# Hypersonic-cpu/DSP-AudioRecLabs

Measured on NVIDIA B200. Metric: audio-seconds processed/sec (features+endpoints+KNN), higher is better.
Workload: dtype i16->f32/f64

## Files before the change

### dsp_audioreclabs_b200/csrc/capi.cu

```cuda
#include <cmath>
#include <cstdarg>
#include <cstdio>
#include <cstdlib>
#include <cstring>
#include <string>
#include <vector>

#include "kernels.cuh"
#include "knn.cuh"
#include "mfcc_dtw.cuh"
#include "misc.cuh"

using namespace dsp;

namespace {

thread_local std::string g_err;

int fail(int code, const char* fmt, ...) {
  char buf[512];
  va_list ap;
  va_start(ap, fmt);
  vsnprintf(buf, sizeof buf, fmt, ap);
  va_end(ap);
  g_err = buf;
  return code;
}

#define CU(expr)                                                                         \
  do {                                                                                   \
    cudaError_t e__ = (expr);                                                            \
    if (e__ != cudaSuccess)                                                              \
      return fail(DSP_ERR_CUDA, "%s failed: %s (%s:%d)", #expr, cudaGetErrorString(e__), \
                  __FILE__, __LINE__);                                                   \
  } while (0)

struct DevBuf {
  void* p = nullptr;
  size_t cap = 0;
  cudaError_t ensure(size_t bytes) {
    if (bytes <= cap) return cudaSuccess;
    if (p) cudaFree(p);
    p = nullptr; cap = 0;
    size_t want = bytes + bytes / 8 + 256;
    cudaError_t e = cudaMalloc(&p, want);
    if (e == cudaSuccess) cap = want;
    return e;
  }
  void release() { if (p) cudaFree(p); p = nullptr; cap = 0; }
  template <class T> T* as() const { return reinterpret_cast<T*>(p); }
};

struct PinBuf {
  void* p = nullptr;
  size_t cap = 0;
  cudaError_t ensure(size_t bytes) {
    if (bytes <= cap) return cudaSuccess;
    if (p) cudaFreeHost(p);
    p = nullptr; cap = 0;
    cudaError_t e = cudaMallocHost(&p, bytes + 256);
    if (e == cudaSuccess) cap = bytes + 256;
    return e;
  }
  void release() { if (p) cudaFreeHost(p); p = nullptr; cap = 0; }
  template <class T> T* as() const { return reinterpret_cast<T*>(p); }
};

constexpr size_t kMaxSmemPerCta = 227 * 1024;
constexpr int64_t kFastMaxLen = 1 << 20;
constexpr int kKnnDenseMaxDim = 16384;
constexpr int64_t kKnnDenseQueryChunk = 32768;
constexpr size_t kHostChunkBytesDefault = 512u << 20;
static size_t host_chunk_bytes() {
  static const size_t v = [] { const char* e = std::getenv("DSP_HOST_CHUNK_MB"); const long mb = e ? std::atol(e) : 0; return mb >= 1 && mb <= 4096 ? (size_t)mb << 20 : kHostChunkBytesDefault; }();
  return v;
}

size_t dtype_size(int dtype) {
  switch (dtype) {
    case DSP_S16: return 2;
    case DSP_U8: return 1;
    case DSP_F32: return 4;
    case DSP_F64: return 8;
    default: return 0;
  }
}

struct Slot {
  DevBuf samples, off, foff, eoff, ints, stats, feat, epd_e, epd_z, f64;
  PinBuf h_off;
  cudaEvent_t ev_in = nullptr, ev_k = nullptr, ev_out = nullptr;
  bool busy = false;
};

}

struct dsp_context {
  int device = 0;
  int sm_count = 0;
  cudaStream_t own = nullptr, stream = nullptr, s_in = nullptr, s_out = nullptr;
  int64_t launches = 0;
  struct WinEntry { int type, len; DevBuf w64, w32; };
  std::vector<WinEntry*> windows;
  const double* win64 = nullptr;
  const float* win32 = nullptr;
  DevBuf counters;
  DevBuf flag_list, zbuf, seqbuf;
  size_t occ_smem = 0;
  int occ_variant = -1;
  int pcm_variant = -1;
  int stagger_ns = 0;
  int tma_chunk = 4096;
  int knn_prune = 1;
  int occ = 0;
  Slot slot[2];
  DevBuf tmp[16];
};

struct dsp_knn {
  dsp_context* ctx = nullptr;
  int64_t n = 0, index_base = 0;
  int d = 0, dp = 0, k = 0;
  float tnorm_max = 0.f;
  bool dense = false;
  bool tc16 = false;
  DevBuf tc_train, tc_train_rows, tc_q, tc_flags;
  DevBuf train64, train32, labels, tnorm, cand_idx, cand_worst, qnorm, redo_list, redo_count, nbr_label, q, o_idx, o_dist, o_lab;
  DevBuf refine_list, refine_thr, surv_count, surv_rows;
  DevBuf thr0;
  DevBuf prune_perm, prune_geom, prune_box, prune_ws, prune_bound;
  int64_t prune_tiles = 0;
  DevBuf tpacked, tnorm_dense, qpacked, qnorm_chunk, dense_flags, part_d, part_i;
};

namespace {

int host_window(int type, int n, std::vector<double>& w) {
  if (n < 0) return fail(DSP_ERR_INVALID, "window length must be >= 0");
  w.assign((size_t)n, 1.0);
  if (type == DSP_WIN_RECTANGULAR) return DSP_OK;
  if (type != DSP_WIN_HAMMING && type != DSP_WIN_HANNING)
    return fail(DSP_ERR_INVALID, "unsupported window type: %d", type);
  if (n <= 1) return DSP_OK;
  const double a = type == DSP_WIN_HAMMING ? 0.54 : 0.5, b = type == DSP_WIN_HAMMING ? 0.46 : 0.5;
  for (int i = 0; i < n; ++i) {
    const double m = (double)(1 - n + 2 * i);
    w[(size_t)i] = a + b * std::cos(M_PI * m / (double)(n - 1));
  }
  return DSP_OK;
}

int ensure_window(dsp_context* c, int type, int fl) {
  for (auto* e : c->windows)
    if (e->type == type && e->len == fl) { c->win64 = e->w64.as<double>(); c->win32 = e->w32.as<float>(); return DSP_OK; }
  std::vector<double> w;
  int rc = host_window(type, fl, w);
  if (rc) return rc;
  std::vector<float> wf(w.begin(), w.end());
  if (c->windows.size() >= 256) {
    CU(cudaDeviceSynchronize());
    for (auto* e : c->windows) { e->w64.release(); e->w32.release(); delete e; }
    c->windows.clear();
  }
  auto* e = new dsp_context::WinEntry{type, fl, {}, {}};
  if (e->w64.ensure(sizeof(double) * (size_t)fl + 16) != cudaSuccess || e->w32.ensure(sizeof(float) * (size_t)fl + 16) != cudaSuccess) {
    e->w64.release(); e->w32.release(); delete e;
    return fail(DSP_ERR_NOMEM, "device allocation failed");
  }
  CU(cudaMemcpy(e->w64.p, w.data(), sizeof(double) * (size_t)fl, cudaMemcpyHostToDevice));
  CU(cudaMemcpy(e->w32.p, wf.data(), sizeof(float) * (size_t)fl, cudaMemcpyHostToDevice));
  c->windows.push_back(e);
  c->win64 = e->w64.as<double>(); c->win32 = e->w32.as<float>();
  return DSP_OK;
}

int check_params(const dsp_frontend_params* p) {
  if (!p) return fail(DSP_ERR_INVALID, "params is NULL");
  if (p->frame_length < 1 || p->frame_shift < 1) return fail(DSP_ERR_INVALID, "frame_length and frame_shift must be >= 1");
  if (p->window < 0 || p->window > 2) return fail(DSP_ERR_INVALID, "unsupported window type: %d", p->window);
  if (p->channels != 1 && p->channels != 2) return fail(DSP_ERR_INVALID, "channels must be 1 or 2 (load_wav only down-mixes two channels, audio_processing.py:43-44: pass other files as 1 channel)");
  return DSP_OK;
}

struct ExactExtras {
  int pre_mode = 3, do_features = 1;
  double* pre_out = nullptr;
  double* frames_out = nullptr;
  double* epd_zcr_f64 = nullptr;
  double* feat_f64[3] = {nullptr, nullptr, nullptr};
  double* stats_f64 = nullptr;
};

int launch_exact(dsp_context* c, const void* samples, int dtype, const int64_t* offsets, const int32_t* lengths,
                 const int64_t* feat_offsets, const int64_t* epd_offsets, const int32_t* list,
                 const int32_t* list_count, int64_t n_items, int64_t max_len, const dsp_frontend_params* p,
                 const dsp_frontend_outputs* out, const ExactExtras& ex, int grid) {
  if (grid < 1) grid = 1;
  const int64_t cap_frames = std::max<int64_t>(frame_count_host_device(max_len, p->frame_length, p->frame_shift), 1);
  CU(c->zbuf.ensure(sizeof(double) * (size_t)grid * (size_t)std::max<int64_t>(max_len, 1)));
  CU(c->seqbuf.ensure(sizeof(double) * (size_t)grid * 5 * (size_t)cap_frames));
  ExactArgs a{};
  a.samples = samples; a.dtype = dtype; a.channels = p->channels;
  a.offsets = offsets; a.lengths = lengths; a.feat_offsets = feat_offsets; a.epd_offsets = epd_offsets;
  a.list = list; a.list_count = list_count; a.n_items = n_items;
  a.fl = p->frame_length; a.fs = p->frame_shift;
  a.do_epd = p->do_endpoint_detection; a.pre_mode = ex.pre_mode; a.do_features = ex.do_features;
  a.hr = p->energy_high_ratio; a.lr = p->energy_low_ratio; a.zr = p->zcr_threshold_ratio;
  a.win = c->win64;
  a.zbuf = c->zbuf.as<double>(); a.zbuf_stride = std::max<int64_t>(max_len, 1);
  a.seqbuf = c->seqbuf.as<double>(); a.seq_cap = cap_frames;
  if (out) a.out = *out;
  a.pre_out = ex.pre_out; a.frames_out = ex.frames_out; a.epd_zcr_f64 = ex.epd_zcr_f64;
  a.feat_f64[0] = ex.feat_f64[0]; a.feat_f64[1] = ex.feat_f64[1]; a.feat_f64[2] = ex.feat_f64[2];
  a.stats_f64 = ex.stats_f64;
  frontend_exact_kernel<<<grid, kExactThreads, 0, c->stream>>>(a);
  c->launches++;
  CU(cudaGetLastError());
  return DSP_OK;
}

int frontend_device(dsp_context* c, const void* samples, int dtype, const int64_t* offsets, const int32_t* lengths,
                    const int64_t* feat_offsets, const int64_t* epd_offsets, int64_t B, int64_t max_len,
                    const dsp_frontend_params* p, const dsp_frontend_outputs* out) {
  int rc = check_params(p);
  if (rc) return rc;
  if (!dtype_size(dtype)) return fail(DSP_ERR_INVALID, "unsupported sample dtype %d", dtype);
  if (!out) return fail(DSP_ERR_INVALID, "outputs is NULL");
  if (B < 0 || max_len < 0) return fail(DSP_ERR_INVALID, "negative batch size or length");
  if (B == 0) return DSP_OK;
  if (B > INT32_MAX / 2) return fail(DSP_ERR_UNSUPPORTED, "more than 2^30 utterances in one call");
  if (p->channels == 2 && (dtype == DSP_F32 || dtype == DSP_F64))
    return fail(DSP_ERR_INVALID, "stereo input is only defined for PCM (load_wav)");
  if ((out->energy || out->magnitude || out->zcr) && !feat_offsets) return fail(DSP_ERR_INVALID, "feat_offsets is NULL");
  if ((out->epd_energy || out->epd_zcr) && !epd_offsets) return fail(DSP_ERR_INVALID, "epd_offsets is NULL");
  rc = ensure_window(c, p->window, p->frame_length);
  if (rc) return rc;
  const int fl = p->frame_length, fs = p->frame_shift;
  const int64_t cap_frames64 = std::max<int64_t>(frame_count_host_device(max_len, fl, fs), 1);

  const bool want64 = out->energy_f64 || out->magnitude_f64 || out->zcr_f64 || out->stats_f64 || out->epd_zcr_f64 || out->frames_f64;
  if (out->frames_f64 && !feat_offsets) return fail(DSP_ERR_INVALID, "feat_offsets is NULL");
  if ((out->energy_f64 || out->magnitude_f64 || out->zcr_f64) && !(out->energy_f64 && out->magnitude_f64 && out->zcr_f64))
    return fail(DSP_ERR_INVALID, "energy_f64, magnitude_f64 and zcr_f64 are written together: pass all three or none");
  if (out->energy_f64 && !feat_offsets) return fail(DSP_ERR_INVALID, "feat_offsets is NULL");
  if (out->epd_zcr_f64 && !epd_offsets) return fail(DSP_ERR_INVALID, "epd_offsets is NULL");
  bool fast = dtype == DSP_S16 && p->channels == 1 && !p->force_exact && !want64 && max_len <= kFastMaxLen &&
              feat_offsets;
  size_t smem = 0;
  int cap_samples = 0;
  constexpr int kAutoStream = 2, kAutoResident = 0;
  int variant = (c->pcm_variant >= 0 && c->pcm_variant < pcm_num_variants()) ? c->pcm_variant : (p->aligned16 ? kAutoStream : kAutoResident);
  if (pcm_variant_streams(variant) && !p->aligned16 && c->pcm_variant < 0) variant = kAutoResident;
  const int kPipeVariant = pcm_num_variants();
  PipePlan plan{};
  bool pipe = fast && (c->pcm_variant == kPipeVariant || c->pcm_variant < 0) &&
              pipe_kernel_plan(max_len, (int)cap_frames64, fl, kMaxSmemPerCta, &plan);
  if (fast && !pipe && c->pcm_variant == kPipeVariant) variant = kAutoResident;
  if (pipe) {
    CU(c->counters.ensure(64));
    CU(c->flag_list.ensure(sizeof(int32_t) * (size_t)B));
    CU(cudaMemsetAsync(c->counters.p, 0, 64, c->stream));
    PcmArgs a{};
    a.samples = reinterpret_cast<const int16_t*>(samples);
    a.offsets = offsets; a.lengths = lengths; a.feat_offsets = feat_offsets; a.epd_offsets = epd_offsets;
    a.n_utts = B; a.fl = fl; a.fs = fs; a.window = p->window; a.do_epd = p->do_endpoint_detection;
    a.hr = p->energy_high_ratio; a.lr = p->energy_low_ratio; a.zr = p->zcr_threshold_ratio;
    a.win_f32 = c->win32;
    a.cap_frames = (int)cap_frames64;
    a.tma_chunk = std::getenv("DSP_PIPE_DEBUG") ? std::atoi(std::getenv("DSP_PIPE_DEBUG")) : 0;
    a.ring_slots = plan.ring_slots; a.n_rec = plan.n_rec; a.cap_groups = plan.cap_groups;
    a.sm_count = c->sm_count;
    a.work_counter = c->counters.as<unsigned int>();
    a.flag_count = c->counters.as<int32_t>() + 1;
    a.flag_list = c->flag_list.as<int32_t>();
    a.out = *out;
    const int grid = (int)std::min<int64_t>(B, (int64_t)c->sm_count);
    static long long* d_prof = nullptr;
    if (std::getenv("DSP_PROF")) {
      if (!d_prof) cudaMalloc(&d_prof, 16 * sizeof(long long));
      cudaMemsetAsync(d_prof, 0, 16 * sizeof(long long), c->stream);
      a.prof = d_prof;
    }
    CU(launch_frontend_pipe(a, grid, plan.smem, c->stream));
    if (a.prof) {
      long long h[16]; cudaMemcpyAsync(h, d_prof, sizeof h, cudaMemcpyDeviceToHost, c->stream); cudaStreamSynchronize(c->stream);
      const char* nm[12] = {"S.wait_full", "S.passA", "S.bar1", "S.passB", "S.bar2", "S.wait_rec", "S.passF", "-", "T.wait", "T.decide", "T.window", "T.stats+out"};
      fprintf(stderr, "[prof pipe R=%d nrec=%d] utterances=%lld (cycles/utt, stream warp 0 / tail warp 0 x nrec)", plan.ring_slots, plan.n_rec, h[15]);
      for (int i = 0; i < 12; ++i) fprintf(stderr, "  %s=%.0f", nm[i], (double)h[i] / (double)std::max<long long>(h[15], 1) * (i >= 8 ? plan.n_rec : 1));
      fprintf(stderr, "\n");
    }
    c->launches++;
    ExactExtras ex;
    const int xgrid = (int)std::min<int64_t>(B, (int64_t)c->sm_count);
    return launch_exact(c, samples, dtype, offsets, lengths, feat_offsets, epd_offsets, a.flag_list, a.flag_count, 0,
                        max_len, p, out, ex, xgrid);
  }
  if (fast) {
    cap_samples = (int)((std::max<int64_t>(max_len, 1) + 63) / 64 * 64);
    smem = pcm_kernel_smem_bytes(cap_samples, (int)cap_frames64, fl, !pcm_variant_streams(variant));
    if (smem > kMaxSmemPerCta && !pcm_variant_streams(variant)) fast = false;
    if (smem > kMaxSmemPerCta) fast = false;
  }
  if (!fast) {
    const int grid = (int)std::min<int64_t>(B, (int64_t)c->sm_count * 4);
    ExactExtras ex;
    ex.feat_f64[0] = out->energy_f64; ex.feat_f64[1] = out->magnitude_f64; ex.feat_f64[2] = out->zcr_f64;
    ex.stats_f64 = out->stats_f64; ex.epd_zcr_f64 = out->epd_zcr_f64; ex.frames_out = out->frames_f64;
    return launch_exact(c, samples, dtype, offsets, lengths, feat_offsets, epd_offsets, nullptr, nullptr, B, max_len,
                        p, out, ex, grid);
  }
  if (c->occ_smem != smem || c->occ_variant != variant) {
    c->occ = pcm_kernel_max_ctas_per_sm(variant, smem);
    c->occ_smem = smem;
    c->occ_variant = variant;
    if (c->occ < 1) return fail(DSP_ERR_CUDA, "fast kernel does not fit: %zu bytes of shared memory", smem);
  }
  CU(c->counters.ensure(64));
  CU(c->flag_list.ensure(sizeof(int32_t) * (size_t)B));
  CU(cudaMemsetAsync(c->counters.p, 0, 64, c->stream));
  PcmArgs a{};
  a.samples = reinterpret_cast<const int16_t*>(samples);
  a.offsets = offsets; a.lengths = lengths; a.feat_offsets = feat_offsets; a.epd_offsets = epd_offsets;
  a.n_utts = B; a.fl = fl; a.fs = fs; a.window = p->window; a.do_epd = p->do_endpoint_detection;
  a.hr = p->energy_high_ratio; a.lr = p->energy_low_ratio; a.zr = p->zcr_threshold_ratio;
  a.win_f32 = c->win32;
  a.cap_samples = cap_samples; a.cap_frames = (int)cap_frames64;
  a.tma_chunk = c->tma_chunk;
  a.stagger_ns = c->stagger_ns;
  a.sm_count = c->sm_count;
  a.prof = nullptr;
  static long long* d_prof = nullptr;
  if (std::getenv("DSP_PROF")) {
    if (!d_prof) cudaMalloc(&d_prof, 16 * sizeof(long long));
    cudaMemsetAsync(d_prof, 0, 16 * sizeof(long long), c->stream);
    a.prof = d_prof;
  }
  a.work_counter = c->counters.as<unsigned int>();
  a.flag_count = c->counters.as<int32_t>() + 1;
  a.flag_list = c->flag_list.as<int32_t>();
  a.out = *out;
  const int grid = (int)std::min<int64_t>(B, (int64_t)c->sm_count * c->occ);
  CU(launch_frontend_pcm(variant, a, grid, smem, c->stream));
  if (a.prof) { long long h[16]; cudaMemcpyAsync(h, d_prof, sizeof h, cudaMemcpyDeviceToHost, c->stream); cudaStreamSynchronize(c->stream);
    const char* nm[12] = {"load_wait", "P1", "feat_empty_wait", "P2", "P2b", "P3tail(searches)", "P4", "fixup+handoff", "P3a(select passes)", "P3b(gather)", "P3c(rank+thresholds)", "P3d(N3N4)"};
    double tot = 0; for (int i = 0; i < 12; ++i) tot += (double)h[i];
    fprintf(stderr, "[prof] utterances=%lld", h[15]); for (int i = 0; i < 12; ++i) fprintf(stderr, "  %s=%.0f", nm[i], (double)h[i] / (double)h[15]); fprintf(stderr, "  total=%.0f cycles/utt\n", tot / (double)h[15]); }
  c->launches++;
  ExactExtras ex;
  const int xgrid = (int)std::min<int64_t>(B, (int64_t)c->sm_count);
  return launch_exact(c, samples, dtype, offsets, lengths, feat_offsets, epd_offsets, a.flag_list, a.flag_count, 0,
                      max_len, p, out, ex, xgrid);
}

struct OneShot {
  dsp_context* c;
  int n_tmp = 0;
  explicit OneShot(dsp_context* ctx) : c(ctx) {}
  template <class T> T* dev(size_t count) {
    DevBuf& b = c->tmp[n_tmp++];
    if (b.ensure(sizeof(T) * std::max<size_t>(count, 1)) != cudaSuccess) return nullptr;
    return b.as<T>();
  }
};

}

extern "C" {

int dsp_abi_version(void) { return DSPFRONT_ABI_VERSION; }
const char* dsp_last_error(void) { return g_err.c_str(); }

int dsp_create(int device, dsp_context** out) {
  if (!out) return fail(DSP_ERR_INVALID, "out is NULL");
  *out = nullptr;
  int count = 0;
  if (cudaGetDeviceCount(&count) != cudaSuccess || count == 0) {
    cudaGetLastError();
    return fail(DSP_ERR_NO_DEVICE, "no CUDA device: libdspfront has no CPU path");
  }
  if (device < 0 || device >= count) return fail(DSP_ERR_INVALID, "device %d out of range (%d visible)", device, count);
  CU(cudaSetDevice(device));
  cudaDeviceProp prop;
  CU(cudaGetDeviceProperties(&prop, device));
  if (prop.major < 10) return fail(DSP_ERR_NO_DEVICE, "device %d is sm_%d%d; this library is built for sm_100a only", device, prop.major, prop.minor);
  dsp_context* c = new dsp_context();
  c->device = device;
  c->sm_count = prop.multiProcessorCount;
  CU(cudaStreamCreateWithFlags(&c->own, cudaStreamNonBlocking));
  CU(cudaStreamCreateWithFlags(&c->s_in, cudaStreamNonBlocking));
  CU(cudaStreamCreateWithFlags(&c->s_out, cudaStreamNonBlocking));
  c->stream = c->own;
  if (const char* e = std::getenv("DSP_PCM_VARIANT")) { int v = std::atoi(e); if (v >= -1 && v <= pcm_num_variants()) c->pcm_variant = v; }
  if (const char* e = std::getenv("DSP_STAGGER_NS")) c->stagger_ns = std::atoi(e);
  if (const char* e = std::getenv("DSP_TMA_CHUNK")) { int v = std::atoi(e); if (v >= 16 && v % 16 == 0) c->tma_chunk = v; }
  for (auto& s : c->slot) {
    CU(cudaEventCreateWithFlags(&s.ev_in, cudaEventDisableTiming));
    CU(cudaEventCreateWithFlags(&s.ev_k, cudaEventDisableTiming));
    CU(cudaEventCreateWithFlags(&s.ev_out, cudaEventDisableTiming));
  }
  *out = c;
  return DSP_OK;
}

int dsp_destroy(dsp_context* c) {
  if (!c) return DSP_OK;
  cudaSetDevice(c->device);
  cudaDeviceSynchronize();
  for (auto& s : c->slot) {
    s.samples.release(); s.off.release(); s.foff.release(); s.eoff.release(); s.ints.release();
    s.stats.release(); s.feat.release(); s.epd_e.release(); s.epd_z.release(); s.f64.release(); s.h_off.release();
    if (s.ev_in) cudaEventDestroy(s.ev_in);
    if (s.ev_k) cudaEventDestroy(s.ev_k);
    if (s.ev_out) cudaEventDestroy(s.ev_out);
  }
  for (auto& b : c->tmp) b.release();
  for (auto* e : c->windows) { e->w64.release(); e->w32.release(); delete e; }
  c->windows.clear();
  c->counters.release(); c->flag_list.release();
  c->zbuf.release(); c->seqbuf.release();
  if (c->own) cudaStreamDestroy(c->own);
  if (c->s_in) cudaStreamDestroy(c->s_in);
  if (c->s_out) cudaStreamDestroy(c->s_out);
  delete c;
  return DSP_OK;
}

int dsp_set_stream(dsp_context* c, void* cuda_stream) {
  if (!c) return fail(DSP_ERR_INVALID, "context is NULL");
  c->stream = reinterpret_cast<cudaStream_t>(cuda_stream);
  return DSP_OK;
}

int dsp_use_own_stream(dsp_context* c) {
  if (!c) return fail(DSP_ERR_INVALID, "context is NULL");
  c->stream = c->own;
  return DSP_OK;
}

int dsp_set_tuning(dsp_context* c, const char* key, int value) {
  if (!c || !key) return fail(DSP_ERR_INVALID, "bad argument");
  if (!std::strcmp(key, "pcm_variant")) {
    if (value < -1 || value > pcm_num_variants()) return fail(DSP_ERR_INVALID, "pcm_variant out of range (%d builds + the pipelined kernel)", pcm_num_variants());
    c->pcm_variant = value;
  } else if (!std::strcmp(key, "tma_chunk")) {
    if (value < 16 || value % 16) return fail(DSP_ERR_INVALID, "tma_chunk must be a positive multiple of 16");
    c->tma_chunk = value;
  } else if (!std::strcmp(key, "stagger_ns")) {
    c->stagger_ns = value;
  } else if (!std::strcmp(key, "knn_prune")) {
    if (value < 0 || value > 2) return fail(DSP_ERR_INVALID, "knn_prune must be 0 (off), 1 (automatic) or 2 (always)");
    c->knn_prune = value;
  } else {
    return fail(DSP_ERR_INVALID, "unknown tuning key '%s'", key);
  }
  return DSP_OK;
}

int dsp_sync(dsp_context* c) {
  if (!c) return fail(DSP_ERR_INVALID, "context is NULL");
  CU(cudaSetDevice(c->device));
  CU(cudaStreamSynchronize(c->stream));
  return DSP_OK;
}

int64_t dsp_launch_count(dsp_context* c) { return c ? c->launches : 0; }
int dsp_device_sm_count(dsp_context* c) { return c ? c->sm_count : 0; }

int64_t dsp_frame_count(int64_t n, int32_t fl, int32_t fs) {
  if (fl < 1 || fs < 1) return 0;
  return frame_count_host_device(n, fl, fs);
}

int dsp_frontend_plan(const int64_t* offsets, const int32_t* lengths, int64_t B, const dsp_frontend_params* p,
                      int64_t* feat_offsets, int64_t* epd_offsets, int64_t* max_len) {
  int rc = check_params(p);
  if (rc) return rc;
  if (!offsets || B < 0) return fail(DSP_ERR_INVALID, "bad offsets");
  int64_t fo = 0, eo = 0, mx = 0;
  for (int64_t b = 0; b < B; ++b) {
    const int64_t room = offsets[b + 1] - offsets[b];
    const int64_t len = lengths ? (int64_t)lengths[b] : room;
    if (room < 0 || len < 0 || len > room || len % p->channels)
      return fail(DSP_ERR_INVALID, "offsets must be non-decreasing, lengths must fit and be a multiple of channels (utterance %lld)", (long long)b);
    const int64_t n = len / p->channels;
    if (n > INT32_MAX / 4) return fail(DSP_ERR_UNSUPPORTED, "utterance %lld is too long", (long long)b);
    if (feat_offsets) feat_offsets[b] = fo;
    if (epd_offsets) epd_offsets[b] = eo;
    fo += frame_count_host_device(n, p->frame_length, p->frame_shift);
    eo += (p->do_endpoint_detection && n >= p->frame_length) ? (n - p->frame_length) / p->frame_shift + 1 : 0;
    mx = std::max(mx, n);
  }
  if (feat_offsets) feat_offsets[B] = fo;
  if (epd_offsets) epd_offsets[B] = eo;
  if (max_len) *max_len = mx;
  return DSP_OK;
}

int dsp_window(int window_type, int32_t length, double* out) {
  std::vector<double> w;
  int rc = host_window(window_type, length, w);
  if (rc) return rc;
  if (length > 0 && !out) return fail(DSP_ERR_INVALID, "out is NULL");
  std::memcpy(out, w.data(), sizeof(double) * w.size());
  return DSP_OK;
}

int dsp_frontend_batch_device(dsp_context* c, const void* samples, int dtype, const int64_t* offsets,
                              const int32_t* lengths, const int64_t* feat_offsets, const int64_t* epd_offsets, int64_t n_utts,
                              int64_t max_len, const dsp_frontend_params* p, const dsp_frontend_outputs* out) {
  if (!c) return fail(DSP_ERR_INVALID, "context is NULL");
  CU(cudaSetDevice(c->device));
  return frontend_device(c, samples, dtype, offsets, lengths, feat_offsets, epd_offsets, n_utts, max_len, p, out);
}

int dsp_frontend_batch_host(dsp_context* c, const void* samples, int dtype, const int64_t* offsets,
                            const int32_t* lengths, int64_t B, const dsp_frontend_params* p, const dsp_frontend_outputs* out) {
  if (!c) return fail(DSP_ERR_INVALID, "context is NULL");
  int rc = check_params(p);
  if (rc) return rc;
  const size_t esz = dtype_size(dtype);
  if (!esz) return fail(DSP_ERR_INVALID, "unsupported sample dtype %d", dtype);
  if (!out || !offsets) return fail(DSP_ERR_INVALID, "NULL argument");
  if (B == 0) return DSP_OK;
  CU(cudaSetDevice(c->device));
  std::vector<int64_t> foff((size_t)B + 1), eoff((size_t)B + 1);
  int64_t max_len_all = 0;
  rc = dsp_frontend_plan(offsets, lengths, B, p, foff.data(), eoff.data(), &max_len_all);
  if (rc) return rc;
  rc = ensure_window(c, p->window, p->frame_length);
  if (rc) return rc;

  const unsigned char* src = reinterpret_cast<const unsigned char*>(samples);
  int64_t b0 = 0;
  int chunk = 0;
  while (b0 < B) {
    int64_t b1 = b0 + 1;
    while (b1 < B && (size_t)(offsets[b1 + 1] - offsets[b0]) * esz <= host_chunk_bytes()) ++b1;
    const int64_t bc = b1 - b0;
    Slot& s = c->slot[chunk & 1];
    if (s.busy) { CU(cudaEventSynchronize(s.ev_out)); s.busy = false; }
    const int64_t e0 = offsets[b0], e1 = offsets[b1];
    const int64_t f0 = foff[(size_t)b0], f1 = foff[(size_t)b1], g0 = eoff[(size_t)b0], g1 = eoff[(size_t)b1];
    CU(s.h_off.ensure(sizeof(int64_t) * 4 * (size_t)(bc + 1)));
    int64_t* h = s.h_off.as<int64_t>();
    int64_t chunk_max = 0;
    for (int64_t i = 0; i <= bc; ++i) {
      h[i] = offsets[b0 + i] - e0;
      h[(bc + 1) + i] = foff[(size_t)(b0 + i)] - f0;
      h[2 * (bc + 1) + i] = eoff[(size_t)(b0 + i)] - g0;
      if (i < bc) {
        const int64_t len = lengths ? (int64_t)lengths[b0 + i] : offsets[b0 + i + 1] - offsets[b0 + i];
        chunk_max = std::max(chunk_max, len / p->channels);
        reinterpret_cast<int32_t*>(h + 3 * (bc + 1))[i] = (int32_t)len;
      }
    }
    CU(s.samples.ensure((size_t)(e1 - e0) * esz + 64));
    CU(s.off.ensure(sizeof(int64_t) * 4 * (size_t)(bc + 1)));
    CU(s.ints.ensure(sizeof(int32_t) * 5 * (size_t)bc));
    CU(s.stats.ensure(sizeof(float) * kStats * (size_t)bc));
    CU(s.feat.ensure(sizeof(float) * 3 * (size_t)std::max<int64_t>(f1 - f0, 1)));
    CU(s.epd_e.ensure(sizeof(double) * (size_t)std::max<int64_t>(g1 - g0, 1)));
    CU(s.epd_z.ensure(sizeof(float) * (size_t)std::max<int64_t>(g1 - g0, 1)));
    const bool want64 = out->energy_f64 || out->magnitude_f64 || out->zcr_f64 || out->stats_f64 || out->epd_zcr_f64 || out->frames_f64;
    const int64_t fn64 = std::max<int64_t>(f1 - f0, 1), gn64 = std::max<int64_t>(g1 - g0, 1);
    const size_t dense64 = out->frames_f64 ? (size_t)fn64 * (size_t)p->frame_length : 0;
    if (want64) CU(s.f64.ensure(sizeof(double) * ((size_t)(3 * fn64 + kStats * bc + gn64) + dense64)));
    CU(cudaMemcpyAsync(s.samples.p, src + (size_t)e0 * esz, (size_t)(e1 - e0) * esz, cudaMemcpyHostToDevice, c->s_in));
    CU(cudaMemcpyAsync(s.off.p, h, sizeof(int64_t) * 4 * (size_t)(bc + 1), cudaMemcpyHostToDevice, c->s_in));
    CU(cudaEventRecord(s.ev_in, c->s_in));
    CU(cudaStreamWaitEvent(c->stream, s.ev_in, 0));
    int32_t* di = s.ints.as<int32_t>();
    float* df = s.feat.as<float>();
    const int64_t fn = std::max<int64_t>(f1 - f0, 1);
    dsp_frontend_outputs o{};
    o.start = di; o.end = di + bc; o.n_epd_frames = di + 2 * bc; o.n_frames = di + 3 * bc; o.status = di + 4 * bc;
    o.energy = df; o.magnitude = df + fn; o.zcr = df + 2 * fn;
    o.stats = s.stats.as<float>();
    o.epd_energy = out->epd_energy ? s.epd_e.as<double>() : nullptr;
    o.epd_zcr = out->epd_zcr ? s.epd_z.as<float>() : nullptr;
    if (want64) {
      double* d64 = s.f64.as<double>();
      if (out->energy_f64) { o.energy_f64 = d64; o.magnitude_f64 = d64 + fn64; o.zcr_f64 = d64 + 2 * fn64; }
      if (out->stats_f64) o.stats_f64 = d64 + 3 * fn64;
      if (out->epd_zcr_f64) o.epd_zcr_f64 = d64 + 3 * fn64 + kStats * bc;
      if (out->frames_f64) o.frames_f64 = d64 + 3 * fn64 + kStats * bc + gn64;
    }
    const int64_t* doff = s.off.as<int64_t>();
    dsp_frontend_params pc = *p;
    pc.aligned16 = 1;
    for (int64_t i = 0; i < bc && pc.aligned16; ++i) if ((size_t)h[i] * esz % 16) pc.aligned16 = 0;
    const int32_t* dlen = lengths ? reinterpret_cast<const int32_t*>(doff + 3 * (bc + 1)) : nullptr;
    rc = frontend_device(c, s.samples.p, dtype, doff, dlen, doff + (bc + 1), doff + 2 * (bc + 1), bc, chunk_max, &pc, &o);
    if (rc) return rc;
    CU(cudaEventRecord(s.ev_k, c->stream));
    CU(cudaStreamWaitEvent(c->s_out, s.ev_k, 0));
    auto d2h = [&](void* dst, const void* srcp, size_t bytes) -> cudaError_t {
      if (!dst || bytes == 0) return cudaSuccess;
      return cudaMemcpyAsync(dst, srcp, bytes, cudaMemcpyDeviceToHost, c->s_out);
    };
    CU(d2h(out->start ? out->start + b0 : nullptr, o.start, sizeof(int32_t) * (size_t)bc));
    CU(d2h(out->end ? out->end + b0 : nullptr, o.end, sizeof(int32_t) * (size_t)bc));
    CU(d2h(out->n_epd_frames ? out->n_epd_frames + b0 : nullptr, o.n_epd_frames, sizeof(int32_t) * (size_t)bc));
    CU(d2h(out->n_frames ? out->n_frames + b0 : nullptr, o.n_frames, sizeof(int32_t) * (size_t)bc));
    CU(d2h(out->status ? out->status + b0 : nullptr, o.status, sizeof(int32_t) * (size_t)bc));
    CU(d2h(out->stats ? out->stats + b0 * kStats : nullptr, o.stats, sizeof(float) * kStats * (size_t)bc));
    CU(d2h(out->energy ? out->energy + f0 : nullptr, o.energy, sizeof(float) * (size_t)(f1 - f0)));
    CU(d2h(out->magnitude ? out->magnitude + f0 : nullptr, o.magnitude, sizeof(float) * (size_t)(f1 - f0)));
    CU(d2h(out->zcr ? out->zcr + f0 : nullptr, o.zcr, sizeof(float) * (size_t)(f1 - f0)));
    CU(d2h(out->epd_energy ? out->epd_energy + g0 : nullptr, o.epd_energy, sizeof(double) * (size_t)(g1 - g0)));
    CU(d2h(out->epd_zcr ? out->epd_zcr + g0 : nullptr, o.epd_zcr, sizeof(float) * (size_t)(g1 - g0)));
    CU(d2h(out->energy_f64 ? out->energy_f64 + f0 : nullptr, o.energy_f64, sizeof(double) * (size_t)(f1 - f0)));
    CU(d2h(out->magnitude_f64 ? out->magnitude_f64 + f0 : nullptr, o.magnitude_f64, sizeof(double) * (size_t)(f1 - f0)));
    CU(d2h(out->zcr_f64 ? out->zcr_f64 + f0 : nullptr, o.zcr_f64, sizeof(double) * (size_t)(f1 - f0)));
    CU(d2h(out->stats_f64 ? out->stats_f64 + b0 * kStats : nullptr, o.stats_f64, sizeof(double) * kStats * (size_t)bc));
    CU(d2h(out->epd_zcr_f64 ? out->epd_zcr_f64 + g0 : nullptr, o.epd_zcr_f64, sizeof(double) * (size_t)(g1 - g0)));
    CU(d2h(out->frames_f64 ? out->frames_f64 + (size_t)f0 * (size_t)p->frame_length : nullptr, o.frames_f64, sizeof(double) * (size_t)(f1 - f0) * (size_t)p->frame_length));
    CU(cudaEventRecord(s.ev_out, c->s_out));
    s.busy = true;
    b0 = b1;
    ++chunk;
  }
  for (auto& s : c->slot)
    if (s.busy) { CU(cudaEventSynchronize(s.ev_out)); s.busy = false; }
  return DSP_OK;
}

static int one_signal(dsp_context* c, const double* x, int64_t n, const dsp_frontend_params* p,
                      const ExactExtras& ex_in, dsp_frontend_outputs* dout, OneShot& os) {
  int rc = ensure_window(c, p->window, p->frame_length);
  if (rc) return rc;
  double* dx = os.dev<double>((size_t)n);
  int64_t* doff = os.dev<int64_t>(2);
  if (!dx || !doff) return fail(DSP_ERR_NOMEM, "device allocation failed");
  const int64_t hoff[2] = {0, n};
  CU(cudaMemcpyAsync(dx, x, sizeof(double) * (size_t)n, cudaMemcpyHostToDevice, c->stream));
  CU(cudaMemcpyAsync(doff, hoff, sizeof hoff, cudaMemcpyHostToDevice, c->stream));
  CU(cudaStreamSynchronize(c->stream));
  return launch_exact(c, dx, DSP_F64, doff, nullptr, nullptr, nullptr, nullptr, nullptr, 1, n, p, dout, ex_in, 1);
}

int dsp_preprocess_host(dsp_context* c, const double* x, int64_t n, int mode, double* out) {
  if (!c || (!x && n) || (!out && n) || n < 0 || mode < 0 || mode > 2) return fail(DSP_ERR_INVALID, "bad argument");
  if (n == 0) return fail(DSP_ERR_INVALID, "zero-size array to reduction operation maximum which has no identity");
  CU(cudaSetDevice(c->device));
  dsp_frontend_params p{};
  p.frame_length = 1; p.frame_shift = 1; p.window = 0; p.channels = 1;
  OneShot os(c);
  double* dout = os.dev<double>((size_t)n);
  if (!dout) return fail(DSP_ERR_NOMEM, "device allocation failed");
  ExactExtras ex;
  ex.pre_mode = mode == 0 ? 1 : (mode == 1 ? 2 : 3);
  ex.do_features = 0;
  ex.pre_out = dout;
  dsp_frontend_outputs o{};
  int rc = one_signal(c, x, n, &p, ex, &o, os);
  if (rc) return rc;
  CU(cudaMemcpyAsync(out, dout, sizeof(double) * (size_t)n, cudaMemcpyDeviceToHost, c->stream));
  CU(cudaStreamSynchronize(c->stream));
  return DSP_OK;
}

int dsp_endpoint_detection_host(dsp_context* c, const double* x, int64_t n, const dsp_frontend_params* p,
                                int32_t* start, int32_t* end, int32_t* n_epd_frames, double* energy_list,
                                double* zcr_list) {
  if (!c || (!x && n) || n < 0) return fail(DSP_ERR_INVALID, "bad argument");
  int rc = check_params(p);
  if (rc) return rc;
  CU(cudaSetDevice(c->device));
  dsp_frontend_params q = *p;
  q.do_endpoint_detection = 1; q.channels = 1; q.window = DSP_WIN_RECTANGULAR;
  const int64_t f1 = n >= q.frame_length ? (n - q.frame_length) / q.frame_shift + 1 : 0;
  OneShot os(c);
  int32_t* di = os.dev<int32_t>(8);
  double* de = os.dev<double>((size_t)f1);
  double* dz = os.dev<double>((size_t)f1);
  if (!di || !de || !dz) return fail(DSP_ERR_NOMEM, "device allocation failed");
  ExactExtras ex;
  ex.pre_mode = 0; ex.do_features = 0; ex.epd_zcr_f64 = dz;
  dsp_frontend_outputs o{};
  o.start = di; o.end = di + 1; o.n_epd_frames = di + 2; o.epd_energy = de;
  rc = one_signal(c, x, n, &q, ex, &o, os);
  if (rc) return rc;
  int32_t hi[3];
  CU(cudaMemcpyAsync(hi, di, sizeof hi, cudaMemcpyDeviceToHost, c->stream));
  if (energy_list && f1) CU(cudaMemcpyAsync(energy_list, de, sizeof(double) * (size_t)f1, cudaMemcpyDeviceToHost, c->stream));
  if (zcr_list && f1) CU(cudaMemcpyAsync(zcr_list, dz, sizeof(double) * (size_t)f1, cudaMemcpyDeviceToHost, c->stream));
  CU(cudaStreamSynchronize(c->stream));
  if (start) *start = hi[0];
  if (end) *end = hi[1];
  if (n_epd_frames) *n_epd_frames = hi[2];
  return DSP_OK;
}

int dsp_frame_signal_host(dsp_context* c, const double* x, int64_t n, int32_t fl, int32_t fs, int window_type,
                          double* frames_out) {
  if (!c || (!x && n) || n < 0) return fail(DSP_ERR_INVALID, "bad argument");
  dsp_frontend_params p{};
  p.frame_length = fl; p.frame_shift = fs; p.window = window_type; p.channels = 1;
  int rc = check_params(&p);
  if (rc) return rc;
  const int64_t nf = frame_count_host_device(n, fl, fs);
  if (nf == 0) return DSP_OK;
  if (!frames_out) return fail(DSP_ERR_INVALID, "frames_out is NULL");
  CU(cudaSetDevice(c->device));
  OneShot os(c);
  double* dfr = os.dev<double>((size_t)nf * (size_t)fl);
  if (!dfr) return fail(DSP_ERR_NOMEM, "device allocation failed");
  ExactExtras ex;
  ex.pre_mode = 0; ex.do_features = 1; ex.frames_out = dfr;
  dsp_frontend_outputs o{};
  rc = one_signal(c, x, n, &p, ex, &o, os);
  if (rc) return rc;
  CU(cudaMemcpyAsync(frames_out, dfr, sizeof(double) * (size_t)nf * (size_t)fl, cudaMemcpyDeviceToHost, c->stream));
  CU(cudaStreamSynchronize(c->stream));
  return DSP_OK;
}

int dsp_frame_features_host(dsp_context* c, const double* frames, int64_t n_frames, int32_t fl, double* energy,
                            double* magnitude, double* zcr, double* stats) {
  if (!c || n_frames < 0 || fl < 0) return fail(DSP_ERR_INVALID, "bad argument");
  if (n_frames == 0) return fail(DSP_ERR_INVALID, "No frames provided for feature extraction.");
  if (n_frames > INT32_MAX) return fail(DSP_ERR_UNSUPPORTED, "too many frames");
  CU(cudaSetDevice(c->device));
  OneShot os(c);
  double* dfr = os.dev<double>((size_t)n_frames * (size_t)fl);
  double* de = os.dev<double>((size_t)n_frames * 3);
  double* dst = os.dev<double>(kStats);
  if (!dfr || !de || !dst) return fail(DSP_ERR_NOMEM, "device allocation failed");
  double* dm = de + n_frames; double* dz = dm + n_frames;
  if (fl > 0) CU(cudaMemcpyAsync(dfr, frames, sizeof(double) * (size_t)n_frames * (size_t)fl, cudaMemcpyHostToDevice, c->stream));
  frame_features_kernel<<<(unsigned)((n_frames + 127) / 128), 128, 0, c->stream>>>(dfr, n_frames, fl, de, dm, dz);
  c->launches++;
  CU(cudaGetLastError());
  if (stats) {
    sequence_stats_kernel<<<1, kExactThreads, 0, c->stream>>>(de, dm, dz, (int)n_frames, dst);
    c->launches++;
    CU(cudaGetLastError());
    CU(cudaMemcpyAsync(stats, dst, sizeof(double) * kStats, cudaMemcpyDeviceToHost, c->stream));
  }
  if (energy) CU(cudaMemcpyAsync(energy, de, sizeof(double) * (size_t)n_frames, cudaMemcpyDeviceToHost, c->stream));
  if (magnitude) CU(cudaMemcpyAsync(magnitude, dm, sizeof(double) * (size_t)n_frames, cudaMemcpyDeviceToHost, c->stream));
  if (zcr) CU(cudaMemcpyAsync(zcr, dz, sizeof(double) * (size_t)n_frames, cudaMemcpyDeviceToHost, c->stream));
  CU(cudaStreamSynchronize(c->stream));
  return DSP_OK;
}

int dsp_sequence_stats_host(dsp_context* c, const double* seq, int64_t n, double* out5) {
  if (!c || !out5 || n < 0) return fail(DSP_ERR_INVALID, "bad argument");
  if (n == 0) return fail(DSP_ERR_INVALID, "zero-size array to reduction operation maximum which has no identity");
  if (n > INT32_MAX) return fail(DSP_ERR_UNSUPPORTED, "sequence too long");
  CU(cudaSetDevice(c->device));
  OneShot os(c);
  double* ds = os.dev<double>((size_t)n);
  double* dst = os.dev<double>(kStats);
  if (!ds || !dst) return fail(DSP_ERR_NOMEM, "device allocation failed");
  CU(cudaMemcpyAsync(ds, seq, sizeof(double) * (size_t)n, cudaMemcpyHostToDevice, c->stream));
  sequence_stats_kernel<<<1, kExactThreads, 0, c->stream>>>(ds, nullptr, nullptr, (int)n, dst);
  c->launches++;
  CU(cudaGetLastError());
  CU(cudaMemcpyAsync(out5, dst, sizeof(double) * 5, cudaMemcpyDeviceToHost, c->stream));
  CU(cudaStreamSynchronize(c->stream));
  return DSP_OK;
}

int dsp_zscore_device(dsp_context* c, const double* x, int64_t n, int32_t d, int fit, double* mean, double* std,
                      double* out) {
  if (!c || n < 0 || d < 1 || !mean || !std) return fail(DSP_ERR_INVALID, "bad argument");
  CU(cudaSetDevice(c->device));
  if (fit) {
    if (n == 0) return fail(DSP_ERR_INVALID, "cannot fit on zero rows");
    CU(zscore_fit(x, n, d, (fit == 2) ? 1 : 0, mean, std, c->stream));
    c->launches++;
  }
  if (out) { CU(zscore_apply(x, n, d, mean, std, out, c->stream)); c->launches += 2; }
  return DSP_OK;
}

int dsp_zscore_apply_f32_device(dsp_context* c, const float* x, int64_t n, int32_t d, const double* mean,
                                const double* std, double* out) {
  if (!c || n < 0 || d < 1 || !mean || !std || (n && (!x || !out))) return fail(DSP_ERR_INVALID, "bad argument");
  CU(cudaSetDevice(c->device));
  CU(zscore_apply_f32(x, n, d, mean, std, out, c->stream));
  c->launches++;
  return DSP_OK;
}

int dsp_zscore_host(dsp_context* c, const double* x, int64_t n, int32_t d, int fit, double* mean, double* std,
                    double* out) {
  if (!c || n < 0 || d < 1 || !mean || !std || (!x && n)) return fail(DSP_ERR_INVALID, "bad argument");
  CU(cudaSetDevice(c->device));
  OneShot os(c);
  double* dx = os.dev<double>((size_t)n * d);
  double* dm = os.dev<double>((size_t)d);
  double* ds = os.dev<double>((size_t)d);
  double* dy = os.dev<double>((size_t)n * d);
  if (!dx || !dm || !ds || !dy) return fail(DSP_ERR_NOMEM, "device allocation failed");
  CU(cudaMemcpyAsync(dx, x, sizeof(double) * (size_t)n * d, cudaMemcpyHostToDevice, c->stream));
  if (!fit) {
    CU(cudaMemcpyAsync(dm, mean, sizeof(double) * d, cudaMemcpyHostToDevice, c->stream));
    CU(cudaMemcpyAsync(ds, std, sizeof(double) * d, cudaMemcpyHostToDevice, c->stream));
  }
  int rc = dsp_zscore_device(c, dx, n, d, fit, dm, ds, out ? dy : nullptr);
  if (rc) return rc;
  CU(cudaMemcpyAsync(mean, dm, sizeof(double) * d, cudaMemcpyDeviceToHost, c->stream));
  CU(cudaMemcpyAsync(std, ds, sizeof(double) * d, cudaMemcpyDeviceToHost, c->stream));
  if (out) CU(cudaMemcpyAsync(out, dy, sizeof(double) * (size_t)n * d, cudaMemcpyDeviceToHost, c->stream));
  CU(cudaStreamSynchronize(c->stream));
  return DSP_OK;
}

static void knn_release(dsp_knn* k) {
  DevBuf* all[] = {&k->train64, &k->train32, &k->labels, &k->tnorm, &k->cand_idx, &k->cand_worst, &k->qnorm,
                   &k->redo_list, &k->redo_count, &k->nbr_label, &k->q, &k->o_idx, &k->o_dist, &k->o_lab,
                   &k->tpacked, &k->tnorm_dense, &k->qpacked, &k->qnorm_chunk, &k->dense_flags, &k->part_d, &k->part_i,
                   &k->tc_train, &k->tc_train_rows, &k->tc_q, &k->tc_flags, &k->refine_list, &k->refine_thr, &k->surv_count, &k->surv_rows, &k->thr0,
                   &k->prune_perm, &k->prune_geom, &k->prune_box, &k->prune_ws, &k->prune_bound};
  for (DevBuf* b : all) b->release();
}

int dsp_knn_fit_device(dsp_context* c, const double* train, const int32_t* labels, int64_t n, int32_t d, int32_t k,
                       int64_t index_base, dsp_knn** out) {
  if (!c || !out || n < 1 || d < 1 || k < 1 || !train || !labels) return fail(DSP_ERR_INVALID, "bad argument");
  if (k > kKnnMaxK) return fail(DSP_ERR_UNSUPPORTED, "n_neighbors > %d is not supported", kKnnMaxK);
  if (n > INT32_MAX) return fail(DSP_ERR_UNSUPPORTED, "more than 2^31 train rows per shard");
  CU(cudaSetDevice(c->device));
  dsp_knn* h = new dsp_knn();
  h->ctx = c; h->n = n; h->d = d; h->k = k; h->index_base = index_base; h->dp = knn_padded_dim(d);
  auto bail = [&](int code) { knn_release(h); delete h; return code; };
  if (h->train64.ensure(sizeof(double) * (size_t)n * d) != cudaSuccess || h->labels.ensure(sizeof(int32_t) * (size_t)n) != cudaSuccess ||
      h->tnorm.ensure(64) != cudaSuccess || h->redo_count.ensure(64) != cudaSuccess)
    return bail(fail(DSP_ERR_NOMEM, "device allocation failed"));
  cudaMemcpyAsync(h->train64.p, train, sizeof(double) * (size_t)n * d, cudaMemcpyDeviceToDevice, c->stream);
  cudaMemcpyAsync(h->labels.p, labels, sizeof(int32_t) * (size_t)n, cudaMemcpyDeviceToDevice, c->stream);
  if (h->dp) {
    if (h->train32.ensure(sizeof(float) * (size_t)n * h->dp) != cudaSuccess) return bail(fail(DSP_ERR_NOMEM, "device allocation failed"));
    cudaError_t e = knn_pack(h->train64.as<double>(), n, d, h->dp, h->train32.as<float>(), h->tnorm.as<float>(), c->stream);
    c->launches++;
    if (e != cudaSuccess) return bail(fail(DSP_ERR_CUDA, "knn_pack: %s", cudaGetErrorString(e)));
    cudaMemcpyAsync(&h->tnorm_max, h->tnorm.p, sizeof(float), cudaMemcpyDeviceToHost, c->stream);
  }
  int tc_flags[2] = {0, 1};
  if (h->dp == 16 && n >= 64 && k < kKnnCand && std::getenv("DSP_KNN_NO_TC16") == nullptr) {
    std::vector<double> host((size_t)n * d);
    if (cudaMemcpyAsync(host.data(), h->train64.p, sizeof(double) * host.size(), cudaMemcpyDeviceToHost, c->stream) != cudaSuccess ||
        cudaStreamSynchronize(c->stream) != cudaSuccess)
      return bail(fail(DSP_ERR_CUDA, "knn fit: %s", cudaGetErrorString(cudaGetLastError())));
    KnnPrunePlan plan;
    knn_prune_plan(host.data(), n, d, plan);
    h->prune_tiles = (int64_t)plan.slack.size();
    const size_t box = sizeof(double) * plan.lo.size();
    if (h->tc_train.ensure(knn_tc16_packed_bytes(n, false)) != cudaSuccess || h->tc_flags.ensure(64) != cudaSuccess ||
        h->prune_perm.ensure(sizeof(int) * (size_t)n) != cudaSuccess || h->prune_geom.ensure(sizeof(KnnPruneGeom)) != cudaSuccess ||
        h->prune_box.ensure(2 * box + sizeof(double) * plan.slack.size()) != cudaSuccess)
      return bail(fail(DSP_ERR_NOMEM, "device allocation failed"));
    unsigned char* pb = h->prune_box.as<unsigned char>();
    cudaMemcpyAsync(h->prune_perm.p, plan.perm.data(), sizeof(int) * (size_t)n, cudaMemcpyHostToDevice, c->stream);
    cudaMemcpyAsync(h->prune_geom.p, &plan.geom, sizeof(KnnPruneGeom), cudaMemcpyHostToDevice, c->stream);
    cudaMemcpyAsync(pb, plan.lo.data(), box, cudaMemcpyHostToDevice, c->stream);
    cudaMemcpyAsync(pb + box, plan.hi.data(), box, cudaMemcpyHostToDevice, c->stream);
    cudaMemcpyAsync(pb + 2 * box, plan.slack.data(), sizeof(double) * plan.slack.size(), cudaMemcpyHostToDevice, c->stream);
    if (h->tc_train_rows.ensure(knn_tc16_packed_bytes(n, false)) != cudaSuccess) return bail(fail(DSP_ERR_NOMEM, "device allocation failed"));
    cudaError_t e = knn_tc16_pack(h->train64.as<double>(), n, d, false, h->tc_train_rows.p, nullptr, h->tc_flags.as<int>(), c->stream);
    if (e == cudaSuccess)
      e = knn_tc16_pack(h->train64.as<double>(), n, d, false, h->tc_train.p, nullptr, h->tc_flags.as<int>(), c->stream,
                        h->prune_perm.as<int>());
    c->launches++;
    if (e != cudaSuccess) return bail(fail(DSP_ERR_CUDA, "knn_tc16_pack: %s", cudaGetErrorString(e)));
    cudaMemcpyAsync(tc_flags, h->tc_flags.p, sizeof tc_flags, cudaMemcpyDeviceToHost, c->stream);
    if (cudaStreamSynchronize(c->stream) != cudaSuccess)
      return bail(fail(DSP_ERR_CUDA, "knn fit: %s", cudaGetErrorString(cudaGetLastError())));
  }
  int dense_flags[2] = {0, 0};
  if (!h->dp && d <= kKnnDenseMaxDim && std::getenv("DSP_KNN_NO_DENSE") == nullptr) {
    if (h->tpacked.ensure(knn_dense_packed_bytes(n, d, true)) != cudaSuccess ||
        h->tnorm_dense.ensure(sizeof(float) * (size_t)knn_dense_padded_rows(n, true)) != cudaSuccess ||
        h->dense_flags.ensure(64) != cudaSuccess)
      return bail(fail(DSP_ERR_NOMEM, "device allocation failed"));
    cudaError_t e = knn_dense_pack(h->train64.as<double>(), n, d, true, h->tpacked.p, h->tnorm_dense.as<float>(), INFINITY,
                                   h->dense_flags.as<int>(), true, c->stream);
    c->launches++;
    if (e != cudaSuccess) return bail(fail(DSP_ERR_CUDA, "knn_dense_pack: %s", cudaGetErrorString(e)));
    cudaMemcpyAsync(dense_flags, h->dense_flags.p, sizeof dense_flags, cudaMemcpyDeviceToHost, c->stream);
  }
  cudaError_t e = cudaStreamSynchronize(c->stream);
  if (e != cudaSuccess) return bail(fail(DSP_ERR_CUDA, "knn fit: %s", cudaGetErrorString(e)));
  h->tc16 = h->tc_train.p && tc_flags[1] == 0;
  if (h->tpacked.p) {
    std::memcpy(&h->tnorm_max, &dense_flags[0], sizeof(float));
    h->dense = dense_flags[1] == 0;
  }
  *out = h;
  return DSP_OK;
}

int dsp_knn_fit_host(dsp_context* c, const double* train, const int32_t* labels, int64_t n, int32_t d, int32_t k,
                     int64_t index_base, dsp_knn** out) {
  if (!c || !out || n < 1 || d < 1 || !train || !labels) return fail(DSP_ERR_INVALID, "bad argument");
  CU(cudaSetDevice(c->device));
  OneShot os(c);
  double* dt = os.dev<double>((size_t)n * d);
  int32_t* dl = os.dev<int32_t>((size_t)n);
  if (!dt || !dl) return fail(DSP_ERR_NOMEM, "device allocation failed");
  CU(cudaMemcpyAsync(dt, train, sizeof(double) * (size_t)n * d, cudaMemcpyHostToDevice, c->stream));
  CU(cudaMemcpyAsync(dl, labels, sizeof(int32_t) * (size_t)n, cudaMemcpyHostToDevice, c->stream));
  return dsp_knn_fit_device(c, dt, dl, n, d, k, index_base, out);
}

int dsp_knn_free(dsp_knn* k) {
  if (!k) return DSP_OK;
  cudaSetDevice(k->ctx->device);
  cudaStreamSynchronize(k->ctx->stream);
  knn_release(k);
  delete k;
  return DSP_OK;
}

int dsp_knn_topk_device(dsp_knn* h, const double* q, int64_t m, int64_t* nbr_idx, double* nbr_sqdist, int32_t* nbr_label) {
  return dsp_knn_topk_bounded_device(h, q, m, nullptr, nbr_idx, nbr_sqdist, nbr_label);
}

int dsp_knn_topk_bounded_device(dsp_knn* h, const double* q, int64_t m, const double* bound, int64_t* nbr_idx, double* nbr_sqdist,
                                int32_t* nbr_label) {
  if (!h || m < 0 || (!q && m)) return fail(DSP_ERR_INVALID, "bad argument");
  if (m == 0) return DSP_OK;
  if (m > INT32_MAX) return fail(DSP_ERR_UNSUPPORTED, "more than 2^31 queries per call");
  dsp_context* c = h->ctx;
  CU(cudaSetDevice(c->device));
  CU(h->redo_list.ensure(sizeof(int32_t) * (size_t)m));
  const unsigned long long* prune_kept = nullptr;
  int64_t prune_visits = 0;
  if (h->dp) {
    CU(h->cand_idx.ensure(sizeof(int) * (size_t)m * kKnnCand));
    CU(h->cand_worst.ensure(sizeof(float) * (size_t)m));
    CU(h->qnorm.ensure(sizeof(float) * (size_t)m));
    double err_rel = (double)(h->d + 4) * 1.1920929e-7, err_floor = 0.0;
    float qnorm_limit = 0.f;
    const float* thr0 = nullptr;
    const double* rerank_bound = nullptr;
    if (h->tc16) {
      CU(h->tc_q.ensure(knn_tc16_packed_bytes(m, true)));
      int* qflags = h->tc_flags.as<int>() + 4;
      err_rel = knn_dense_err_rel(16);
      err_floor = 1.0;
      qnorm_limit = knn_tc16_max_norm();
      Tc16Work work;
      const void* tpacked = h->tc_train_rows.p;
      const bool prune = c->knn_prune && knn_tc16_padded_rows(m, true) / kTc16UnitQueries * h->prune_tiles <= INT32_MAX;
      if (prune) {
        CU(h->prune_ws.ensure(knn_prune_scratch_bytes(m, h->n)));
        CU(h->prune_bound.ensure(sizeof(double) * (size_t)m));
        CU(h->thr0.ensure(sizeof(float) * (size_t)m));
        const unsigned char* pb = h->prune_box.as<unsigned char>();
        const size_t box = sizeof(double) * (size_t)h->prune_tiles * h->d;
        CU(knn_prune_prepare(q, m, h->n, h->d, h->k, h->train64.as<double>(), h->prune_geom.as<KnnPruneGeom>(), h->prune_perm.as<int>(),
                             (const double*)pb, (const double*)(pb + box), (const double*)(pb + 2 * box), h->tc_train.p, h->tc_q.p,
                             h->qnorm.as<float>(), qflags, bound, h->prune_bound.as<double>(), h->cand_idx.as<int>(),
                             h->cand_worst.as<float>(), h->prune_ws.p, c->knn_prune == 1, c->sm_count, c->stream, work));
        tpacked = h->tc_train.p;
        rerank_bound = h->prune_bound.as<double>();
        prune_kept = work.kept;
        prune_visits = knn_tc16_padded_rows(m, true) / kTc16UnitQueries * h->prune_tiles;
        CU(knn_bound_thresholds(rerank_bound, h->qnorm.as<float>(), m, err_rel, err_floor, h->thr0.as<float>(), c->stream));
        thr0 = h->thr0.as<float>();
        c->launches += 12;
      } else {
        CU(knn_tc16_pack(q, m, h->d, true, h->tc_q.p, h->qnorm.as<float>(), qflags, c->stream));
      }
      if (bound && !prune) {
        CU(h->thr0.ensure(sizeof(float) * (size_t)m));
        CU(knn_bound_thresholds(bound, h->qnorm.as<float>(), m, err_rel, err_floor, h->thr0.as<float>(), c->stream));
        thr0 = h->thr0.as<float>();
        rerank_bound = bound;
        c->launches += 1;
      }
      CU(knn_tc16_filter(h->tc_q.p, tpacked, m, h->n, h->k, qflags, h->cand_idx.as<int>(), h->cand_worst.as<float>(),
                         c->sm_count, c->stream, thr0, work));
      c->launches += 2;
    } else {
      CU(knn_scan(h->dp, h->train32.as<float>(), h->n, q, m, h->d, h->cand_idx.as<int>(), h->cand_worst.as<float>(),
                  h->qnorm.as<float>(), nullptr, c->stream));
      c->launches += 1;
    }
    const int refine_cap = (h->dp == 16 && h->k < kKnnCand) ? (int)std::min<int64_t>(m, 65536) : 0;
    if (refine_cap) {
      CU(h->refine_list.ensure(sizeof(int32_t) * (size_t)refine_cap));
      CU(h->refine_thr.ensure(sizeof(float) * (size_t)refine_cap));
      CU(h->surv_count.ensure(sizeof(int32_t) * (size_t)refine_cap));
      CU(h->surv_rows.ensure(sizeof(int32_t) * (size_t)refine_cap * knn_refine_survivor_cap()));
    }
    CU(knn_rerank(h->train64.as<double>(), h->train32.as<float>(), h->dp, h->n, q, m, h->d, h->k, h->index_base,
                  h->labels.as<int32_t>(), h->cand_idx.as<int>(), h->cand_worst.as<float>(), h->qnorm.as<float>(),
                  h->tnorm_max, err_rel, err_floor, nbr_idx, nbr_sqdist, nbr_label, h->redo_list.as<int32_t>(),
                  h->redo_count.as<int32_t>(), c->stream, refine_cap ? h->refine_list.as<int32_t>() : nullptr,
                  h->refine_thr.as<float>(), refine_cap, qnorm_limit, rerank_bound, thr0, bound && thr0));
    c->launches += 1;
    if (refine_cap) {
      CU(knn_refine(h->train64.as<double>(), h->train32.as<float>(), h->dp, h->n, q, h->d, h->k, h->index_base,
                    h->labels.as<int32_t>(), h->refine_list.as<int32_t>(), h->refine_thr.as<float>(), refine_cap,
                    h->surv_count.as<int32_t>(), h->surv_rows.as<int32_t>(), h->redo_count.as<int32_t>(),
                    h->redo_list.as<int32_t>(), nbr_idx, nbr_sqdist, nbr_label, c->sm_count, c->stream, bound && thr0));
      c->launches += 2;
    }
  } else if (h->dense) {
    CU(h->cand_idx.ensure(sizeof(int) * (size_t)m * kKnnCand));
    CU(h->cand_worst.ensure(sizeof(float) * (size_t)m));
    CU(h->qnorm.ensure(sizeof(float) * (size_t)m));
    const int64_t chunk = std::min<int64_t>(m, kKnnDenseQueryChunk);
    CU(h->qpacked.ensure(knn_dense_packed_bytes(chunk, h->d, false)));
    CU(h->qnorm_chunk.ensure(sizeof(float) * (size_t)knn_dense_padded_rows(chunk, false)));
    CU(h->dense_flags.ensure(64));
    for (int64_t q0 = 0; q0 < m; q0 += chunk) {
      const int64_t mc = std::min<int64_t>(chunk, m - q0);
      CU(knn_dense_pack(q + q0 * h->d, mc, h->d, false, h->qpacked.p, h->qnorm_chunk.as<float>(), 0.f, h->dense_flags.as<int>(),
                        q0 == 0, c->stream));
      CU(cudaMemcpyAsync(h->qnorm.as<float>() + q0, h->qnorm_chunk.p, sizeof(float) * (size_t)mc, cudaMemcpyDeviceToDevice, c->stream));
      CU(knn_dense_scan(h->qpacked.p, h->tpacked.p, h->tnorm_dense.as<float>(), mc, h->n, h->d,
                        h->cand_idx.as<int>() + q0 * kKnnCand, h->cand_worst.as<float>() + q0, c->sm_count, c->stream));
      c->launches += 2;
    }
    int qflags[2] = {0, 0};
    CU(cudaMemcpyAsync(qflags, h->dense_flags.p, sizeof qflags, cudaMemcpyDeviceToHost, c->stream));
    CU(cudaStreamSynchronize(c->stream));
    const bool all_fit = qflags[1] == 0;
    if (all_fit) {
      CU(knn_rerank(h->train64.as<double>(), nullptr, 0, h->n, q, m, h->d, h->k, h->index_base,
                    h->labels.as<int32_t>(), h->cand_idx.as<int>(), h->cand_worst.as<float>(), h->qnorm.as<float>(),
                    h->tnorm_max, knn_dense_err_rel(h->d), 0.0, nbr_idx, nbr_sqdist, nbr_label, h->redo_list.as<int32_t>(),
                    h->redo_count.as<int32_t>(), c->stream));
    } else {
      CU(knn_redo_all(h->redo_list.as<int32_t>(), h->redo_count.as<int32_t>(), m, c->stream));
    }
    c->launches++;
  } else {
    CU(knn_redo_all(h->redo_list.as<int32_t>(), h->redo_count.as<int32_t>(), m, c->stream));
    c->launches++;
  }
  CU(h->part_d.ensure(sizeof(double) * (size_t)knn_rescan_grid(c->sm_count) * kKnnMaxK));
  CU(h->part_i.ensure(sizeof(long long) * (size_t)knn_rescan_grid(c->sm_count) * kKnnMaxK));
  CU(knn_rescan(h->train64.as<double>(), h->n, q, h->d, h->k, h->index_base, h->labels.as<int32_t>(),
                h->redo_list.as<int32_t>(), h->redo_count.as<int32_t>(), nbr_idx, nbr_sqdist, nbr_label,
                c->sm_count, h->part_d.as<double>(), h->part_i.as<long long>(), (int)std::min<int64_t>(m, INT32_MAX), c->stream));
  c->launches++;
  if (std::getenv("DSP_KNN_DEBUG")) {
    int32_t cnt[4];
    cudaMemcpyAsync(cnt, h->redo_count.p, sizeof cnt, cudaMemcpyDeviceToHost, c->stream);
    cudaStreamSynchronize(c->stream);
    fprintf(stderr, "[knn] m=%lld n=%lld exhaustive=%d refined=%d refined->exhaustive=%d\n", (long long)m, (long long)h->n, cnt[0], cnt[1], cnt[2]);
    if (prune_kept) {
      unsigned long long kept = 0;
      cudaMemcpyAsync(&kept, prune_kept, sizeof kept, cudaMemcpyDeviceToHost, c->stream);
      cudaStreamSynchronize(c->stream);
      fprintf(stderr, "[knn] prune: tile visits kept=%llu of %lld (%s)\n", kept, (long long)prune_visits,
              c->knn_prune == 1 && kept > (unsigned long long)(0.85 * (double)prune_visits) ? "every tile walked" : "lists walked");
    }
  }
  return DSP_OK;
}

int dsp_mfcc_batch_host(dsp_context* c, const int16_t* samples, const int64_t* offsets, const int32_t* lengths,
                        const int32_t* seg_start, const int32_t* seg_end, int64_t n_utts, const dsp_mfcc_params* p,
                        const float* filterbank, const float* dct, const int64_t* mfcc_offsets, float* mfcc_out,
                        int32_t* n_frames_out) {
  if (!c || !p || n_utts < 0 || (n_utts && (!samples || !offsets || !seg_start || !seg_end || !filterbank || !dct || !mfcc_offsets || !mfcc_out)))
    return fail(DSP_ERR_INVALID, "bad argument");
  if (p->frame_length < 1 || p->frame_shift < 1 || p->n_mels < 1 || p->n_ceps < 1 || p->n_ceps > p->n_mels)
    return fail(DSP_ERR_INVALID, "bad MFCC geometry");
  if (p->n_fft < 32 || (p->n_fft & (p->n_fft - 1)) || p->n_fft < p->frame_length || p->n_fft > 16384)
    return fail(DSP_ERR_INVALID, "n_fft must be a power of two in [max(32, frame_length), 16384]");
  if (mfcc_smem_bytes(p->n_fft, p->n_mels) > kMaxSmemPerCta) return fail(DSP_ERR_UNSUPPORTED, "n_fft too large for shared memory");
  if (n_utts == 0) return DSP_OK;
  CU(cudaSetDevice(c->device));
  std::vector<double> w;
  int rc = host_window(p->window, p->frame_length, w);
  if (rc) return rc;
  std::vector<float> wf(w.begin(), w.end());
  const int n_bins = p->n_fft / 2 + 1;
  std::vector<float> tw((size_t)p->n_fft);
  for (int k = 0; k < p->n_fft / 2; ++k) {
    const double a = -2.0 * M_PI * (double)k / (double)p->n_fft;
    tw[2 * (size_t)k] = (float)std::cos(a); tw[2 * (size_t)k + 1] = (float)std::sin(a);
  }
  std::vector<int> range(2 * (size_t)p->n_mels);
  for (int m = 0; m < p->n_mels; ++m) {
    int lo = n_bins, hi = 0;
    for (int b = 0; b < n_bins; ++b) if (filterbank[(size_t)m * n_bins + b] != 0.f) { lo = std::min(lo, b); hi = std::max(hi, b + 1); }
    range[2 * (size_t)m] = std::min(lo, hi); range[2 * (size_t)m + 1] = hi;
  }
  const int64_t total_samples = lengths ? offsets[n_utts - 1] + lengths[n_utts - 1] : offsets[n_utts];
  int64_t span = 0;
  for (int64_t b = 0; b < n_utts; ++b) span = std::max<int64_t>(span, offsets[b] + (lengths ? lengths[b] : offsets[b + 1] - offsets[b]));
  const int64_t total_frames = mfcc_offsets[n_utts];
  (void)total_samples;
  OneShot os(c);
  int16_t* d_s = os.dev<int16_t>((size_t)span);
  int64_t* d_off = os.dev<int64_t>((size_t)n_utts + 1);
  int32_t* d_len = lengths ? os.dev<int32_t>((size_t)n_utts) : nullptr;
  int32_t* d_st = os.dev<int32_t>((size_t)n_utts);
  int32_t* d_en = os.dev<int32_t>((size_t)n_utts);
  float* d_w = os.dev<float>(wf.size());
  float* d_tw = os.dev<float>(tw.size());
  float* d_fb = os.dev<float>((size_t)p->n_mels * n_bins);
  int* d_rg = os.dev<int>(range.size());
  float* d_dct = os.dev<float>((size_t)p->n_ceps * p->n_mels);
  int64_t* d_mo = os.dev<int64_t>((size_t)n_utts + 1);
  float* d_out = os.dev<float>((size_t)std::max<int64_t>(total_frames, 1) * p->n_ceps);
  int32_t* d_nf = os.dev<int32_t>((size_t)n_utts);
  unsigned int* d_cnt = os.dev<unsigned int>(4);
  if (!d_s || !d_off || (lengths && !d_len) || !d_st || !d_en || !d_w || !d_tw || !d_fb || !d_rg || !d_dct || !d_mo || !d_out || !d_nf || !d_cnt)
    return fail(DSP_ERR_NOMEM, "device allocation failed");
  cudaStream_t st = c->stream;
  CU(cudaMemcpyAsync(d_s, samples, sizeof(int16_t) * (size_t)span, cudaMemcpyHostToDevice, st));
  CU(cudaMemcpyAsync(d_off, offsets, sizeof(int64_t) * ((size_t)n_utts + 1), cudaMemcpyHostToDevice, st));
  if (lengths) CU(cudaMemcpyAsync(d_len, lengths, sizeof(int32_t) * (size_t)n_utts, cudaMemcpyHostToDevice, st));
  CU(cudaMemcpyAsync(d_st, seg_start, sizeof(int32_t) * (size_t)n_utts, cudaMemcpyHostToDevice, st));
  CU(cudaMemcpyAsync(d_en, seg_end, sizeof(int32_t) * (size_t)n_utts, cudaMemcpyHostToDevice, st));
  CU(cudaMemcpyAsync(d_w, wf.data(), sizeof(float) * wf.size(), cudaMemcpyHostToDevice, st));
  CU(cudaMemcpyAsync(d_tw, tw.data(), sizeof(float) * tw.size(), cudaMemcpyHostToDevice, st));
  CU(cudaMemcpyAsync(d_fb, filterbank, sizeof(float) * (size_t)p->n_mels * n_bins, cudaMemcpyHostToDevice, st));
  CU(cudaMemcpyAsync(d_rg, range.data(), sizeof(int) * range.size(), cudaMemcpyHostToDevice, st));
  CU(cudaMemcpyAsync(d_dct, dct, sizeof(float) * (size_t)p->n_ceps * p->n_mels, cudaMemcpyHostToDevice, st));
  CU(cudaMemcpyAsync(d_mo, mfcc_offsets, sizeof(int64_t) * ((size_t)n_utts + 1), cudaMemcpyHostToDevice, st));
  MfccArgs a{p->frame_length, p->frame_shift, p->n_fft, p->n_mels, p->n_ceps, p->pre_emphasis, (float)p->log_floor};
  CU(launch_mfcc(d_s, d_off, d_len, d_st, d_en, n_utts, a, d_w, reinterpret_cast<const float2*>(d_tw), d_fb,
                 reinterpret_cast<const int2*>(d_rg), d_dct, d_mo, d_out, d_nf, d_cnt, c->sm_count, st));
  c->launches++;
  if (total_frames > 0) CU(cudaMemcpyAsync(mfcc_out, d_out, sizeof(float) * (size_t)total_frames * p->n_ceps, cudaMemcpyDeviceToHost, st));
  if (n_frames_out) CU(cudaMemcpyAsync(n_frames_out, d_nf, sizeof(int32_t) * (size_t)n_utts, cudaMemcpyDeviceToHost, st));
  CU(cudaStreamSynchronize(st));
  return DSP_OK;
}

int dsp_dtw_topk_host(dsp_context* c, const float* q_feats, const int64_t* q_offsets, int64_t nq, const float* t_feats,
                      const int64_t* t_offsets, const int32_t* t_labels, int64_t nt, int32_t dim, int32_t k,
                      int64_t index_base, float* cost_out, double* nbr_cost, int64_t* nbr_idx, int32_t* nbr_label) {
  if (!c || nq < 0 || nt < 1 || dim < 1 || k < 1 || !q_offsets || !t_offsets || (nq && !q_feats) || !t_feats || (nbr_label && !t_labels))
    return fail(DSP_ERR_INVALID, "bad argument");
  if (k > kKnnMaxK) return fail(DSP_ERR_UNSUPPORTED, "k > %d is not supported", kKnnMaxK);
  if (dim > dtw_max_dim()) return fail(DSP_ERR_UNSUPPORTED, "feature dimension > %d is not supported by the DTW kernel", dtw_max_dim());
  if (nq == 0) return DSP_OK;
  int64_t max_q = 0, max_t = 0;
  for (int64_t i = 0; i < nq; ++i) max_q = std::max(max_q, q_offsets[i + 1] - q_offsets[i]);
  for (int64_t i = 0; i < nt; ++i) max_t = std::max(max_t, t_offsets[i + 1] - t_offsets[i]);
  if (max_q > dtw_max_query_frames()) return fail(DSP_ERR_UNSUPPORTED, "query sequences longer than %d frames are not supported", dtw_max_query_frames());
  if (dtw_smem_bytes((int)max_t, dim) > kMaxSmemPerCta) return fail(DSP_ERR_UNSUPPORTED, "template sequence too long for shared memory (%lld frames x %d features)", (long long)max_t, dim);
  CU(cudaSetDevice(c->device));
  OneShot os(c);
  float* d_q = os.dev<float>((size_t)q_offsets[nq] * dim);
  int64_t* d_qo = os.dev<int64_t>((size_t)nq + 1);
  float* d_t = os.dev<float>((size_t)t_offsets[nt] * dim);
  int64_t* d_to = os.dev<int64_t>((size_t)nt + 1);
  int32_t* d_lab = os.dev<int32_t>((size_t)nt);
  float* d_cost = os.dev<float>((size_t)nq * nt);
  double* d_nc = os.dev<double>((size_t)nq * k);
  int64_t* d_ni = os.dev<int64_t>((size_t)nq * k);
  int32_t* d_nl = os.dev<int32_t>((size_t)nq * k);
  if (!d_q || !d_qo || !d_t || !d_to || !d_lab || !d_cost || !d_nc || !d_ni || !d_nl) return fail(DSP_ERR_NOMEM, "device allocation failed");
  cudaStream_t st = c->stream;
  CU(cudaMemcpyAsync(d_q, q_feats, sizeof(float) * (size_t)q_offsets[nq] * dim, cudaMemcpyHostToDevice, st));
  CU(cudaMemcpyAsync(d_qo, q_offsets, sizeof(int64_t) * ((size_t)nq + 1), cudaMemcpyHostToDevice, st));
  CU(cudaMemcpyAsync(d_t, t_feats, sizeof(float) * (size_t)t_offsets[nt] * dim, cudaMemcpyHostToDevice, st));
  CU(cudaMemcpyAsync(d_to, t_offsets, sizeof(int64_t) * ((size_t)nt + 1), cudaMemcpyHostToDevice, st));
  if (t_labels) CU(cudaMemcpyAsync(d_lab, t_labels, sizeof(int32_t) * (size_t)nt, cudaMemcpyHostToDevice, st));
  else CU(cudaMemsetAsync(d_lab, 0, sizeof(int32_t) * (size_t)nt, st));
  CU(launch_dtw(d_q, d_qo, nq, (int)max_q, d_t, d_to, nt, (int)max_t, dim, d_cost, st));
  CU(launch_dtw_topk(d_cost, nq, nt, k, index_base, d_lab, d_nc, d_ni, d_nl, st));
  c->launches += 2;
  if (cost_out) CU(cudaMemcpyAsync(cost_out, d_cost, sizeof(float) * (size_t)nq * nt, cudaMemcpyDeviceToHost, st));
  if (nbr_cost) CU(cudaMemcpyAsync(nbr_cost, d_nc, sizeof(double) * (size_t)nq * k, cudaMemcpyDeviceToHost, st));
  if (nbr_idx) CU(cudaMemcpyAsync(nbr_idx, d_ni, sizeof(int64_t) * (size_t)nq * k, cudaMemcpyDeviceToHost, st));
  if (nbr_label) CU(cudaMemcpyAsync(nbr_label, d_nl, sizeof(int32_t) * (size_t)nq * k, cudaMemcpyDeviceToHost, st));
  CU(cudaStreamSynchronize(st));
  return DSP_OK;
}

int dsp_knn_last_stats(dsp_knn* h, int64_t* rescanned, int32_t* scan_kind) {
  if (!h) return fail(DSP_ERR_INVALID, "bad argument");
  CU(cudaSetDevice(h->ctx->device));
  int32_t cnt[4] = {0, 0, 0, 0};
  if (h->redo_count.p) {
    CU(cudaMemcpyAsync(cnt, h->redo_count.p, sizeof cnt, cudaMemcpyDeviceToHost, h->ctx->stream));
    CU(cudaStreamSynchronize(h->ctx->stream));
  }
  if (rescanned) *rescanned = (int64_t)cnt[0] + cnt[1] - cnt[2];
  if (scan_kind) *scan_kind = h->dp ? (h->tc16 ? 3 : 1) : (h->dense ? 2 : 0);
  return DSP_OK;
}

int dsp_knn_predict_device(dsp_knn* h, const double* q, int64_t m, int32_t* labels_out) {
  if (!h || !labels_out) return fail(DSP_ERR_INVALID, "bad argument");
  if (m == 0) return DSP_OK;
  dsp_context* c = h->ctx;
  CU(cudaSetDevice(c->device));
  CU(h->nbr_label.ensure(sizeof(int32_t) * (size_t)m * h->k));
  int rc = dsp_knn_topk_device(h, q, m, nullptr, nullptr, h->nbr_label.as<int32_t>());
  if (rc) return rc;
  CU(knn_vote(h->nbr_label.as<int32_t>(), m, h->k, labels_out, c->stream));
  c->launches++;
  return DSP_OK;
}

int dsp_knn_topk_host(dsp_knn* h, const double* q, int64_t m, int64_t* nbr_idx, double* nbr_sqdist, int32_t* nbr_label) {
  if (!h || m < 0 || (!q && m)) return fail(DSP_ERR_INVALID, "bad argument");
  if (m == 0) return DSP_OK;
  dsp_context* c = h->ctx;
  CU(cudaSetDevice(c->device));
  CU(h->q.ensure(sizeof(double) * (size_t)m * h->d));
  CU(h->o_idx.ensure(sizeof(int64_t) * (size_t)m * h->k));
  CU(h->o_dist.ensure(sizeof(double) * (size_t)m * h->k));
  CU(h->o_lab.ensure(sizeof(int32_t) * (size_t)m * h->k));
  CU(cudaMemcpyAsync(h->q.p, q, sizeof(double) * (size_t)m * h->d, cudaMemcpyHostToDevice, c->stream));
  int rc = dsp_knn_topk_device(h, h->q.as<double>(), m, h->o_idx.as<int64_t>(), h->o_dist.as<double>(), h->o_lab.as<int32_t>());
  if (rc) return rc;
  if (nbr_idx) CU(cudaMemcpyAsync(nbr_idx, h->o_idx.p, sizeof(int64_t) * (size_t)m * h->k, cudaMemcpyDeviceToHost, c->stream));
  if (nbr_sqdist) CU(cudaMemcpyAsync(nbr_sqdist, h->o_dist.p, sizeof(double) * (size_t)m * h->k, cudaMemcpyDeviceToHost, c->stream));
  if (nbr_label) CU(cudaMemcpyAsync(nbr_label, h->o_lab.p, sizeof(int32_t) * (size_t)m * h->k, cudaMemcpyDeviceToHost, c->stream));
  CU(cudaStreamSynchronize(c->stream));
  return DSP_OK;
}

int dsp_knn_predict_host(dsp_knn* h, const double* q, int64_t m, int32_t* labels_out) {
  if (!h || !labels_out || m < 0 || (!q && m)) return fail(DSP_ERR_INVALID, "bad argument");
  if (m == 0) return DSP_OK;
  dsp_context* c = h->ctx;
  CU(cudaSetDevice(c->device));
  CU(h->q.ensure(sizeof(double) * (size_t)m * h->d));
  CU(h->o_lab.ensure(sizeof(int32_t) * (size_t)m));
  CU(cudaMemcpyAsync(h->q.p, q, sizeof(double) * (size_t)m * h->d, cudaMemcpyHostToDevice, c->stream));
  int rc = dsp_knn_predict_device(h, h->q.as<double>(), m, h->o_lab.as<int32_t>());
  if (rc) return rc;
  CU(cudaMemcpyAsync(labels_out, h->o_lab.p, sizeof(int32_t) * (size_t)m, cudaMemcpyDeviceToHost, c->stream));
  CU(cudaStreamSynchronize(c->stream));
  return DSP_OK;
}

int dsp_knn_merge_vote_device(dsp_context* c, const double* cand_sqdist, const int64_t* cand_idx, const int32_t* cand_label,
                              int32_t n_lists, int64_t m, int32_t k, int32_t* labels_out, int64_t* nbr_idx_out,
                              double* nbr_sqdist_out) {
  if (!c || !cand_sqdist || !cand_idx || !cand_label || n_lists < 1 || m < 0 || k < 1 || k > kKnnMaxK)
    return fail(DSP_ERR_INVALID, "bad argument");
  CU(cudaSetDevice(c->device));
  CU(knn_merge_vote(cand_sqdist, cand_idx, cand_label, n_lists, m, k, labels_out, nbr_idx_out, nbr_sqdist_out, c->stream));
  c->launches++;
  return DSP_OK;
}

}
```

### dsp_audioreclabs_b200/csrc/knn.cuh

```cuda
#pragma once
#include <cuda_runtime.h>
#include <stdint.h>

#include <vector>

namespace dsp {

constexpr int kKnnCand = 8;
constexpr int kKnnMaxK = 16;

int knn_padded_dim(int d);
cudaError_t knn_pack(const double* train, int64_t n, int d, int dp, float* train32, float* tnorm_max,
                     cudaStream_t st);
cudaError_t knn_scan(int dp, const float* train32, int64_t n, const double* q, int64_t m, int d,
                     int* cand_idx, float* cand_worst, float* qnorm, const int* gate, cudaStream_t st);
cudaError_t knn_rerank(const double* train, const float* train32, int dp, int64_t n, const double* q,
                       int64_t m, int d, int k, int64_t index_base, const int32_t* labels,
                       const int* cand_idx, const float* cand_worst, const float* qnorm,
                       float tnorm_max_host, double err_rel, double err_floor, int64_t* nbr_idx, double* nbr_sqdist, int32_t* nbr_label,
                       int32_t* redo_list, int32_t* redo_count, cudaStream_t st, int32_t* refine_list = nullptr,
                       float* refine_thr = nullptr, int refine_cap = 0, float qnorm_limit = 0.f,
                       const double* bound = nullptr, const float* thr0 = nullptr, bool allow_short = true);
int knn_refine_survivor_cap();
cudaError_t knn_refine(const double* train, const float* train32, int dp, int64_t n, const double* q, int d, int k,
                       int64_t index_base, const int32_t* labels, const int32_t* refine_list, const float* refine_thr,
                       int refine_cap, int32_t* surv_count, int32_t* surv_rows, int32_t* counts, int32_t* redo_list,
                       int64_t* nbr_idx, double* nbr_sqdist, int32_t* nbr_label, int sm_count, cudaStream_t st,
                       bool allow_short = false);
cudaError_t knn_redo_all(int32_t* redo_list, int32_t* redo_count, int64_t m, cudaStream_t st);
cudaError_t knn_rescan(const double* train, int64_t n, const double* q, int d, int k, int64_t index_base,
                       const int32_t* labels, const int32_t* redo_list, const int32_t* redo_count,
                       int64_t* nbr_idx, double* nbr_sqdist, int32_t* nbr_label, int sm_count,
                       double* part_d, long long* part_i, int max_redo, cudaStream_t st);
int knn_rescan_grid(int sm_count);
cudaError_t knn_vote(const int32_t* nbr_label, int64_t m, int k, int32_t* out, cudaStream_t st);
cudaError_t knn_merge_vote(const double* cd, const int64_t* ci, const int32_t* cl, int r, int64_t m,
                           int k, int32_t* labels_out, int64_t* idx_out, double* dist_out,
                           cudaStream_t st);

float knn_tc16_max_norm();
int64_t knn_tc16_padded_rows(int64_t rows, bool query);
size_t knn_tc16_packed_bytes(int64_t rows, bool query);
constexpr int kTc16TileRows = 128;
constexpr int kTc16UnitQueries = 256;
cudaError_t knn_tc16_pack(const double* x, int64_t rows, int d, bool query, void* packed, float* norms, int* flags, cudaStream_t st,
                          const int* gather = nullptr);
struct Tc16Work {
  const int* tiles = nullptr;
  const int* tile_count = nullptr;
  int stride = 0;
  const int* unit_order = nullptr;
  int* counter = nullptr;
  const unsigned long long* kept = nullptr;
  unsigned long long kept_limit = 0;
  const int* qperm = nullptr;
  const int* tperm = nullptr;
};
cudaError_t knn_tc16_filter(const void* qpacked, const void* tpacked, int64_t m, int64_t n, int k, const int* qflags, int* cand_idx,
                            float* cand_worst, int sm_count, cudaStream_t st, const float* thr0 = nullptr, const Tc16Work& work = Tc16Work());

constexpr int kPruneMaxDim = 15;
constexpr int kPruneSeedTiles = 4;
struct KnnPruneGeom {
  int d;
  double mean[kPruneMaxDim];
  double axis[kPruneMaxDim][kPruneMaxDim];
  double key_lo[3], key_scale[3];
};
struct KnnPrunePlan {
  KnnPruneGeom geom;
  std::vector<int> perm;
  std::vector<double> lo, hi, slack;
};
void knn_prune_plan(const double* train, int64_t n, int d, KnnPrunePlan& plan);
size_t knn_prune_scratch_bytes(int64_t m, int64_t n);
cudaError_t knn_prune_prepare(const double* q, int64_t m, int64_t n, int d, int k, const double* train, const KnnPruneGeom* geom,
                              const int* tperm, const double* tile_lo, const double* tile_hi, const double* tile_slack, const void* tpacked,
                              void* qpacked, float* qnorm, int* qflags, const double* caller_bound, double* bound, int* cand_idx,
                              float* cand_worst, void* scratch, bool auto_fallback, int sm_count, cudaStream_t st, Tc16Work& work);
cudaError_t knn_bound_thresholds(const double* bound, const float* qnorm, int64_t m, double err_rel, double err_floor, float* thr0,
                                 cudaStream_t st);

int knn_dense_kblocks(int d);
int64_t knn_dense_padded_rows(int64_t rows, bool train);
size_t knn_dense_packed_bytes(int64_t rows, int d, bool train);
cudaError_t knn_dense_pack(const double* x, int64_t rows, int d, bool train, void* packed, float* norms, float pad_norm,
                           int* flags, bool reset_flags, cudaStream_t st);
cudaError_t knn_dense_scan(const void* qpacked, const void* tpacked, const float* tnorm, int64_t m, int64_t n, int d,
                           int* cand_idx, float* cand_worst, int sm_count, cudaStream_t st);
inline double knn_dense_err_rel(int d) { return (3.0 * d / 16.0 + 32.0) * 2.384185791015625e-07; }

}
```

### dsp_audioreclabs_b200/csrc/knn_tc16.cu

```cuda
#include <cuda_fp16.h>

#include <algorithm>
#include <climits>
#include <cmath>
#include <cstdlib>
#include <cstring>
#include <numeric>

#include <cub/block/block_scan.cuh>
#include <cub/device/device_radix_sort.cuh>

#include "kernels.cuh"
#include "knn.cuh"

namespace dsp {

namespace {

constexpr int kRows = 128;
constexpr int kK = 16;
constexpr int kPlaneBytes = kRows * kK * 2;
constexpr int kTileBytes = 2 * kPlaneBytes;
constexpr int kUnitQ = 2 * kRows;
constexpr int kQBufBytes = 2 * kTileBytes;
#ifndef DSP_TC16_SPLIT
#define DSP_TC16_SPLIT 2
#endif
constexpr int kSplit = DSP_TC16_SPLIT;
constexpr int kTStages = kSplit == 1 ? 18 : 16;
constexpr int kAccStages = kSplit == 4 ? 4 : 2;
constexpr int kMmaN = kSplit == 4 ? 64 : kRows;
constexpr int kEpiWarps = kSplit == 1 ? 8 : 16;
constexpr int kTcThreads = 32 * (2 + kEpiWarps);
constexpr int kTmemCols = 512;
constexpr int kEpiThreads = 32 * kEpiWarps;
constexpr int kListBytes = 2 * kKnnCand * kEpiThreads * 4;
constexpr size_t kTcSmem = 2 * kQBufBytes + (size_t)kTStages * kTileBytes + kListBytes + 1024;
constexpr uint32_t kLBO = 128, kSBO = 256;
constexpr uint32_t kIdesc = (1u << 4) | ((uint32_t)(kMmaN >> 3) << 17) | ((uint32_t)(kRows >> 4) << 24);
static_assert(8 * (4 + 2 * kTStages + 2 * kAccStages) + 8 <= 512, "barrier block of the shared-memory plan (unit slots at 512)");
constexpr float kPadNorm = 30000.f;

__device__ __forceinline__ uint32_t smem_u32(const void* p) { return (uint32_t)__cvta_generic_to_shared(p); }
__device__ __forceinline__ void mbar_init(uint64_t* bar, int count) {
  asm volatile("mbarrier.init.shared::cta.b64 [%0], %1;" ::"r"(smem_u32(bar)), "r"(count));
}
__device__ __forceinline__ void mbar_expect_tx(uint64_t* bar, uint32_t bytes) {
  asm volatile("mbarrier.arrive.expect_tx.shared::cta.b64 _, [%0], %1;" ::"r"(smem_u32(bar)), "r"(bytes) : "memory");
}
__device__ __forceinline__ void mbar_arrive(uint64_t* bar) {
  asm volatile("mbarrier.arrive.shared::cta.b64 _, [%0];" ::"r"(smem_u32(bar)) : "memory");
}
__device__ __forceinline__ void mbar_wait(uint64_t* bar, uint32_t parity) {
  asm volatile(
      "{\n\t.reg .pred p;\n\t"
      "WAIT_%=:\n\t"
      "mbarrier.try_wait.parity.shared::cta.b64 p, [%0], %1, %2;\n\t"
      "@p bra DONE_%=;\n\t"
      "bra WAIT_%=;\n\t"
      "DONE_%=:\n\t}" ::"r"(smem_u32(bar)), "r"(parity), "r"(0x989680u)
      : "memory");
}
__device__ __forceinline__ void mbar_wait_spin(uint64_t* bar, uint32_t parity) {
  asm volatile(
      "{\n\t.reg .pred p;\n\t"
      "WAIT_%=:\n\t"
      "mbarrier.try_wait.parity.shared::cta.b64 p, [%0], %1;\n\t"
      "@p bra DONE_%=;\n\t"
      "bra WAIT_%=;\n\t"
      "DONE_%=:\n\t}" ::"r"(smem_u32(bar)), "r"(parity)
      : "memory");
}
__device__ __forceinline__ void bulk_g2s(uint32_t dst, const void* src, uint32_t bytes, uint64_t* bar) {
  asm volatile("cp.async.bulk.shared::cluster.global.mbarrier::complete_tx::bytes [%0], [%1], %2, [%3];" ::"r"(dst), "l"(src),
               "r"(bytes), "r"(smem_u32(bar))
               : "memory");
}
__device__ __forceinline__ void tc_fence_before() { asm volatile("tcgen05.fence::before_thread_sync;" ::: "memory"); }
__device__ __forceinline__ void tc_fence_after() { asm volatile("tcgen05.fence::after_thread_sync;" ::: "memory"); }
__device__ __forceinline__ uint64_t umma_desc(uint32_t saddr) {
  return (uint64_t)((saddr >> 4) & 0x3fffu) | ((uint64_t)(kLBO >> 4) << 16) | ((uint64_t)(kSBO >> 4) << 32) | (1ull << 46);
}
__device__ __forceinline__ void umma_f16(uint32_t d_tmem, uint64_t adesc, uint64_t bdesc, uint32_t accumulate) {
  asm volatile(
      "{\n\t.reg .pred p;\n\t"
      "setp.ne.b32 p, %4, 0;\n\t"
      "tcgen05.mma.cta_group::1.kind::f16 [%0], %1, %2, %3, p;\n\t}" ::"r"(d_tmem),
      "l"(adesc), "l"(bdesc), "r"(kIdesc), "r"(accumulate)
      : "memory");
}
__device__ __forceinline__ void umma_commit(uint64_t* bar) {
  asm volatile("tcgen05.commit.cta_group::1.mbarrier::arrive::one.shared::cluster.b64 [%0];" ::"r"(smem_u32(bar)) : "memory");
}
__device__ __forceinline__ void tmem_ld32(uint32_t taddr, uint32_t (&v)[32]) {
  asm volatile(
      "tcgen05.ld.sync.aligned.32x32b.x32.b32 "
      "{%0, %1, %2, %3, %4, %5, %6, %7, %8, %9, %10, %11, %12, %13, %14, %15, "
      "%16, %17, %18, %19, %20, %21, %22, %23, %24, %25, %26, %27, %28, %29, %30, %31}, [%32];"
      : "=r"(v[0]), "=r"(v[1]), "=r"(v[2]), "=r"(v[3]), "=r"(v[4]), "=r"(v[5]), "=r"(v[6]), "=r"(v[7]), "=r"(v[8]),
        "=r"(v[9]), "=r"(v[10]), "=r"(v[11]), "=r"(v[12]), "=r"(v[13]), "=r"(v[14]), "=r"(v[15]), "=r"(v[16]),
        "=r"(v[17]), "=r"(v[18]), "=r"(v[19]), "=r"(v[20]), "=r"(v[21]), "=r"(v[22]), "=r"(v[23]), "=r"(v[24]),
        "=r"(v[25]), "=r"(v[26]), "=r"(v[27]), "=r"(v[28]), "=r"(v[29]), "=r"(v[30]), "=r"(v[31])
      : "r"(taddr)
      : "memory");
}
__device__ __forceinline__ void tmem_ld8(uint32_t taddr, uint32_t (&v)[8]) {
  asm volatile("tcgen05.ld.sync.aligned.32x32b.x8.b32 {%0, %1, %2, %3, %4, %5, %6, %7}, [%8];"
               : "=r"(v[0]), "=r"(v[1]), "=r"(v[2]), "=r"(v[3]), "=r"(v[4]), "=r"(v[5]), "=r"(v[6]), "=r"(v[7])
               : "r"(taddr)
               : "memory");
}
__device__ __forceinline__ void tmem_ld_wait() { asm volatile("tcgen05.wait::ld.sync.aligned;" ::: "memory"); }

__device__ __forceinline__ float min3f(float a, float b, float c) { return fminf(fminf(a, b), c); }
__device__ __forceinline__ float min8(const uint32_t* v) {
  const float a = min3f(__uint_as_float(v[0]), __uint_as_float(v[1]), __uint_as_float(v[2]));
  const float b = min3f(__uint_as_float(v[3]), __uint_as_float(v[4]), __uint_as_float(v[5]));
  return fminf(min3f(a, b, __uint_as_float(v[6])), __uint_as_float(v[7]));
}

__device__ __forceinline__ int plane_offset(int r, int c) { return (r >> 3) * (int)kSBO + (c >> 3) * (int)kLBO + (r & 7) * 16 + (c & 7) * 2; }

__global__ void knn_tc16_pack_kernel(const double* __restrict__ x, int64_t rows, int64_t rows_padded, int d, bool is_query,
                                     unsigned char* __restrict__ packed, float* __restrict__ norms, int* __restrict__ flags,
                                     float max_norm, const int* __restrict__ gather) {
  const int64_t r = (int64_t)blockIdx.x * blockDim.x + threadIdx.x;
  bool bad = false;
  float nf = 0.f;
  if (r < rows_padded) {
    const int64_t src = (r < rows && gather) ? gather[r] : r;
    double v[kK];
    double ss = 0.0;
#pragma unroll
    for (int c = 0; c < kK - 1; ++c) {
      v[c] = (r < rows && c < d) ? x[src * d + c] : 0.0;
      ss += v[c] * v[c];
    }
    bad = r < rows && !(ss <= (double)max_norm);
    nf = (float)ss;
    if (is_query) {
#pragma unroll
      for (int c = 0; c < kK - 1; ++c) v[c] *= -2.0;
      v[kK - 1] = 1.0;
    } else {
      v[kK - 1] = r < rows ? ss : (double)kPadNorm;
    }
    if (bad) {
#pragma unroll
      for (int c = 0; c < kK; ++c) v[c] = 0.0;
    }
    __align__(16) __half hi[kK];
    __align__(16) __half lo[kK];
#pragma unroll
    for (int c = 0; c < kK; ++c) {
      const __half h = __float2half_rn((float)v[c]);
      hi[c] = h;
      lo[c] = __float2half_rn((float)(v[c] - (double)__half2float(h)));
    }
    unsigned char* tile = packed + (size_t)(r / kRows) * kTileBytes;
    const int rr = (int)(r % kRows);
#pragma unroll
    for (int c8 = 0; c8 < 2; ++c8) {
      *reinterpret_cast<uint4*>(tile + plane_offset(rr, 8 * c8)) = *reinterpret_cast<const uint4*>(hi + 8 * c8);
      *reinterpret_cast<uint4*>(tile + kPlaneBytes + plane_offset(rr, 8 * c8)) = *reinterpret_cast<const uint4*>(lo + 8 * c8);
    }
    if (norms && r < rows) norms[src] = nf;
  }
  if (r >= rows) nf = 0.f;
  nf = warp_reduce(bad ? 0.f : nf, [](float a, float b) { return fmaxf(a, b); });
  bad = __any_sync(0xffffffffu, bad);
  if ((threadIdx.x & 31) == 0) {
    atomicMax(&flags[0], __float_as_int(nf));
    if (bad) atomicOr(&flags[1], 1);
  }
}

__device__ __forceinline__ void tmem_ld64(uint32_t taddr, uint32_t (&v)[64]) {
  asm volatile(
      "tcgen05.ld.sync.aligned.32x32b.x64.b32 "
      "{%0, %1, %2, %3, %4, %5, %6, %7, %8, %9, %10, %11, %12, %13, %14, %15, "
      "%16, %17, %18, %19, %20, %21, %22, %23, %24, %25, %26, %27, %28, %29, %30, %31, "
      "%32, %33, %34, %35, %36, %37, %38, %39, %40, %41, %42, %43, %44, %45, %46, %47, "
      "%48, %49, %50, %51, %52, %53, %54, %55, %56, %57, %58, %59, %60, %61, %62, %63}, [%64];"
      : "=r"(v[0]), "=r"(v[1]), "=r"(v[2]), "=r"(v[3]), "=r"(v[4]), "=r"(v[5]), "=r"(v[6]), "=r"(v[7]), "=r"(v[8]),
        "=r"(v[9]), "=r"(v[10]), "=r"(v[11]), "=r"(v[12]), "=r"(v[13]), "=r"(v[14]), "=r"(v[15]), "=r"(v[16]),
        "=r"(v[17]), "=r"(v[18]), "=r"(v[19]), "=r"(v[20]), "=r"(v[21]), "=r"(v[22]), "=r"(v[23]), "=r"(v[24]),
        "=r"(v[25]), "=r"(v[26]), "=r"(v[27]), "=r"(v[28]), "=r"(v[29]), "=r"(v[30]), "=r"(v[31]), "=r"(v[32]),
        "=r"(v[33]), "=r"(v[34]), "=r"(v[35]), "=r"(v[36]), "=r"(v[37]), "=r"(v[38]), "=r"(v[39]), "=r"(v[40]),
        "=r"(v[41]), "=r"(v[42]), "=r"(v[43]), "=r"(v[44]), "=r"(v[45]), "=r"(v[46]), "=r"(v[47]), "=r"(v[48]),
        "=r"(v[49]), "=r"(v[50]), "=r"(v[51]), "=r"(v[52]), "=r"(v[53]), "=r"(v[54]), "=r"(v[55]), "=r"(v[56]),
        "=r"(v[57]), "=r"(v[58]), "=r"(v[59]), "=r"(v[60]), "=r"(v[61]), "=r"(v[62]), "=r"(v[63])
      : "r"(taddr)
      : "memory");
}

template <int C>
__device__ __noinline__ float tc16_slow8(float v0, float v1, float v2, float v3, float v4, float v5, float v6, float v7, int idx0,
                                         float thr, float* __restrict__ l_cd, int* __restrict__ l_ci) {
  const float v[8] = {v0, v1, v2, v3, v4, v5, v6, v7};
#pragma unroll
  for (int j = 0; j < 8; ++j) {
    const float d = v[j];
    if (d < thr) {
      float cd[C]; int ci[C]; bool p[C];
#pragma unroll
      for (int s = 0; s < C; ++s) { cd[s] = l_cd[s * kEpiThreads]; ci[s] = l_ci[s * kEpiThreads]; p[s] = d < cd[s]; }
#pragma unroll
      for (int s = C - 1; s > 0; --s) {
        l_ci[s * kEpiThreads] = p[s] ? (p[s - 1] ? ci[s - 1] : idx0 + j) : ci[s];
        l_cd[s * kEpiThreads] = fminf(fmaxf(cd[s - 1], d), cd[s]);
      }
      l_ci[0] = p[0] ? idx0 + j : ci[0];
      l_cd[0] = fminf(cd[0], d);
      thr = fminf(fmaxf(cd[C - 2], d), cd[C - 1]);
    }
  }
  return thr;
}

template <int kDebug, int kC>
__global__ void __launch_bounds__(kTcThreads, 1)
knn_tc16_filter_kernel(const unsigned char* __restrict__ qpacked, const unsigned char* __restrict__ tpacked, int64_t m, int n,
                       int units, int t_tiles, const int* __restrict__ qflags, int* __restrict__ cand_idx,
                       float* __restrict__ cand_worst, const float* __restrict__ thr0, const Tc16Work w) {
  extern __shared__ __align__(1024) unsigned char smem[];
  unsigned char* s_q = smem;
  unsigned char* s_t = smem + 2 * kQBufBytes;
  uint64_t* bars = reinterpret_cast<uint64_t*>(smem + 2 * kQBufBytes + (size_t)kTStages * kTileBytes);
  uint64_t* q_full = bars;
  uint64_t* q_empty = q_full + 2;
  uint64_t* t_full = q_empty + 2;
  uint64_t* t_empty = t_full + kTStages;
  uint64_t* acc_full = t_empty + kTStages;
  uint64_t* acc_empty = acc_full + kAccStages;
  uint32_t* tmem_slot = reinterpret_cast<uint32_t*>(acc_empty + kAccStages);
  int4* s_info = reinterpret_cast<int4*>(reinterpret_cast<unsigned char*>(bars) + 512);
  const int tid = threadIdx.x, warp = tid >> 5, lane = tid & 31;
  auto wait = [](uint64_t* bar, uint32_t parity) { mbar_wait(bar, parity); };
  auto wait_epi = [](uint64_t* bar, uint32_t parity) { if constexpr (kDebug & 1) mbar_wait_spin(bar, parity); else mbar_wait(bar, parity); };

  if (tid == 0) {
    for (int i = 0; i < 2; ++i) { mbar_init(&q_full[i], 1); mbar_init(&q_empty[i], 1 + kEpiWarps); }
    for (int i = 0; i < kTStages; ++i) { mbar_init(&t_full[i], 1); mbar_init(&t_empty[i], 1); }
    for (int i = 0; i < kAccStages; ++i) { mbar_init(&acc_full[i], 1); mbar_init(&acc_empty[i], kEpiWarps); }
    asm volatile("fence.mbarrier_init.release.cluster;" ::: "memory");
  }
  if (warp == 1) {
    asm volatile("tcgen05.alloc.cta_group::1.sync.aligned.shared::cta.b32 [%0], %1;" ::"r"(smem_u32(tmem_slot)), "r"((uint32_t)kTmemCols) : "memory");
    asm volatile("tcgen05.relinquish_alloc_permit.cta_group::1.sync.aligned;" ::: "memory");
  }
  tc_fence_before();
  __syncthreads();
  tc_fence_after();
  const uint32_t tmem_base = *tmem_slot;

  if (warp == 0) {
    if (lane == 0) {
      int s = 0; uint32_t ph = 0;
      int qb = 0; uint32_t qph = 0;
      const bool lists = w.tiles && !(w.kept && *w.kept > w.kept_limit);
      for (int i = 0;; ++i) {
        wait(&q_empty[qb], qph ^ 1u);
        const int slot = w.counter ? atomicAdd(w.counter, 1) : (int)blockIdx.x + i * (int)gridDim.x;
        const int u = slot < units ? (w.unit_order ? w.unit_order[slot] : slot) : -1;
        const int cnt = (u >= 0 && lists) ? w.tile_count[u] : t_tiles, list = (u >= 0 && lists) ? u * w.stride : -1;
        s_info[qb] = make_int4(u, cnt, list, 0);
        if (u < 0) { mbar_arrive(&q_full[qb]); break; }
        mbar_expect_tx(&q_full[qb], (uint32_t)kQBufBytes);
        bulk_g2s(smem_u32(s_q + (size_t)qb * kQBufBytes), qpacked + (size_t)u * kQBufBytes, kQBufBytes, &q_full[qb]);
        if (++qb == 2) { qb = 0; qph ^= 1u; }
        int tb = cnt > 0 ? (list < 0 ? 0 : w.tiles[list]) : 0;
        for (int j = 0; j < cnt; ++j) {
          const int tb_next = j + 1 < cnt ? (list < 0 ? j + 1 : w.tiles[list + j + 1]) : 0;
          wait(&t_empty[s], ph ^ 1u);
          mbar_expect_tx(&t_full[s], (uint32_t)kTileBytes);
          bulk_g2s(smem_u32(s_t + (size_t)s * kTileBytes), tpacked + (size_t)tb * kTileBytes, kTileBytes, &t_full[s]);
          if (++s == kTStages) { s = 0; ph ^= 1u; }
          tb = tb_next;
        }
      }
    }
    __syncwarp();
  } else if (warp == 1) {
    if (lane == 0) {
      int s = 0, as = 0, qb = 0; uint32_t ph = 0, aph = 0, qph = 0;
      for (;;) {
        wait(&q_full[qb], qph);
        tc_fence_after();
        const int4 info = s_info[qb];
        if (info.x < 0) break;
        const uint32_t q0 = smem_u32(s_q + (size_t)qb * kQBufBytes);
        for (int tb = 0; tb < info.y; ++tb) {
          if constexpr (kSplit == 4) {
            wait(&t_full[s], ph);
            const uint32_t t_base = smem_u32(s_t + (size_t)s * kTileBytes);
#pragma unroll
            for (int sub = 0; sub < 2; ++sub) {
              wait(&acc_empty[as], aph ^ 1u);
              tc_fence_after();
              const uint32_t t_hi = t_base + (uint32_t)sub * (kMmaN / 8) * kSBO, t_lo = t_hi + kPlaneBytes;
#pragma unroll
              for (int h = 0; h < 2; ++h) {
                const uint32_t q_hi = q0 + (uint32_t)h * kTileBytes, q_lo = q_hi + kPlaneBytes;
                const uint32_t d_tmem = tmem_base + (uint32_t)(as * 2 * kMmaN + h * kMmaN);
                umma_f16(d_tmem, umma_desc(q_hi), umma_desc(t_hi), 0u);
                umma_f16(d_tmem, umma_desc(q_hi), umma_desc(t_lo), 1u);
                umma_f16(d_tmem, umma_desc(q_lo), umma_desc(t_hi), 1u);
              }
              if (sub == 1) umma_commit(&t_empty[s]);
              umma_commit(&acc_full[as]);
              if (++as == kAccStages) { as = 0; aph ^= 1u; }
            }
            if (++s == kTStages) { s = 0; ph ^= 1u; }
            continue;
          }
          wait(&acc_empty[as], aph ^ 1u);
          wait(&t_full[s], ph);
          tc_fence_after();
          const uint32_t t_hi = smem_u32(s_t + (size_t)s * kTileBytes), t_lo = t_hi + kPlaneBytes;
#pragma unroll
          for (int h = 0; h < 2; ++h) {
            const uint32_t q_hi = q0 + (uint32_t)h * kTileBytes, q_lo = q_hi + kPlaneBytes;
            const uint32_t d_tmem = tmem_base + (uint32_t)((as * 2 + h) * kRows);
            umma_f16(d_tmem, umma_desc(q_hi), umma_desc(t_hi), 0u);
            umma_f16(d_tmem, umma_desc(q_hi), umma_desc(t_lo), 1u);
            umma_f16(d_tmem, umma_desc(q_lo), umma_desc(t_hi), 1u);
          }
          umma_commit(&t_empty[s]);
          umma_commit(&acc_full[as]);
          if (++s == kTStages) { s = 0; ph ^= 1u; }
          if (++as == kAccStages) { as = 0; aph ^= 1u; }
        }
        umma_commit(&q_empty[qb]);
        if (++qb == 2) { qb = 0; qph ^= 1u; }
      }
    }
    __syncwarp();
  } else {
    const int lg = warp & 3, grp = (warp - 2) >> 2;
    const int h = kSplit == 1 ? grp : grp >> 1, half = kSplit == 1 ? 0 : grp & 1;
    const int et = tid - 64;
    float* l_cd = reinterpret_cast<float*>(smem + 2 * kQBufBytes + (size_t)kTStages * kTileBytes + 1024) + et;
    int* l_ci = reinterpret_cast<int*>(l_cd - et + kKnnCand * kEpiThreads) + et;
    const uint32_t lane_addr = tmem_base + ((uint32_t)(lg * 32) << 16);
    int as = 0, qb = 0; uint32_t aph = 0, qph = 0;
    for (;;) {
      wait_epi(&q_full[qb], qph);
      const int4 info = s_info[qb];
      __syncwarp();
      if (lane == 0) mbar_arrive(&q_empty[qb]);
      if (++qb == 2) { qb = 0; qph ^= 1u; }
      const int u = info.x, cnt = info.y, list = info.z;
      if (u < 0) break;
      auto tile_row = [&](int j) { return (list < 0 ? j : w.tiles[list + j]) * kRows; };
#pragma unroll
      for (int c = 0; c < kKnnCand; ++c) { l_cd[c * kEpiThreads] = INFINITY; l_ci[c * kEpiThreads] = -1; }
      const int64_t q_own = (int64_t)u * kUnitQ + h * kRows + lg * 32 + lane;
      const int64_t q_idx = q_own < m ? (w.qperm ? (int64_t)w.qperm[q_own] : q_own) : -1;
      const float thr_cap = (thr0 && q_idx >= 0) ? thr0[q_idx] : INFINITY;
      float thr = thr_cap;
      auto process = [&](const uint32_t* v, int idx0) {
        if constexpr (kDebug & 2) { if (__uint_as_float(v[0]) == 12345.678f) thr = 0.f; return; }
        const float s0 = min8(v), s1 = min8(v + 8), s2 = min8(v + 16), s3 = min8(v + 24);
        if (fminf(fminf(s0, s1), fminf(s2, s3)) < thr) {
#define DSP_TC16_GROUP(g, sg)                                                                                                     \
          if (sg < thr)                                                                                                          \
            thr = fminf(thr_cap, tc16_slow8<kC>(__uint_as_float(v[8 * g]), __uint_as_float(v[8 * g + 1]), __uint_as_float(v[8 * g + 2]), \
                                 __uint_as_float(v[8 * g + 3]), __uint_as_float(v[8 * g + 4]), __uint_as_float(v[8 * g + 5]),        \
                                 __uint_as_float(v[8 * g + 6]), __uint_as_float(v[8 * g + 7]), idx0 + 8 * g, thr, l_cd, l_ci));
          DSP_TC16_GROUP(0, s0) DSP_TC16_GROUP(1, s1) DSP_TC16_GROUP(2, s2) DSP_TC16_GROUP(3, s3)
#undef DSP_TC16_GROUP
        }
        __syncwarp();
      };
      if constexpr (kSplit == 1) {
        uint32_t va[64], vb[64];
        if (cnt > 0) {
          wait_epi(&acc_full[as], aph);
          tc_fence_after();
          tmem_ld64(lane_addr + (uint32_t)((as * 2 + h) * kRows), va);
        }
        for (int tb = 0; tb < cnt; ++tb) {
          const int base = tile_row(tb);
          tmem_ld_wait();
          tmem_ld64(lane_addr + (uint32_t)((as * 2 + h) * kRows + 64), vb);
          process(va, base);
          process(va + 32, base + 32);
          tmem_ld_wait();
          tc_fence_before();
          __syncwarp();
          if (lane == 0) mbar_arrive(&acc_empty[as]);
          if (++as == kAccStages) { as = 0; aph ^= 1u; }
          if (tb + 1 < cnt) {
            wait_epi(&acc_full[as], aph);
            tc_fence_after();
            tmem_ld64(lane_addr + (uint32_t)((as * 2 + h) * kRows), va);
          }
          process(vb, base + 64);
          process(vb + 32, base + 96);
        }
      } else if constexpr (kSplit == 4) {
        uint32_t va[32], vb[32];
        auto stage_col = [&](int st) { return (uint32_t)(st * 2 * kMmaN + h * kMmaN + half * 32); };
        if (cnt > 0) {
          wait_epi(&acc_full[as], aph);
          tc_fence_after();
          tmem_ld32(lane_addr + stage_col(as), va);
        }
        for (int tb = 0; tb < cnt; ++tb) {
          const int base = tile_row(tb) + half * 32;
          tmem_ld_wait();
          tc_fence_before();
          __syncwarp();
          if (lane == 0) mbar_arrive(&acc_empty[as]);
          if (++as == kAccStages) { as = 0; aph ^= 1u; }
          wait_epi(&acc_full[as], aph);
          tc_fence_after();
          tmem_ld32(lane_addr + stage_col(as), vb);
          process(va, base);
          tmem_ld_wait();
          tc_fence_before();
          __syncwarp();
          if (lane == 0) mbar_arrive(&acc_empty[as]);
          if (++as == kAccStages) { as = 0; aph ^= 1u; }
          if (tb + 1 < cnt) {
            wait_epi(&acc_full[as], aph);
            tc_fence_after();
            tmem_ld32(lane_addr + stage_col(as), va);
          }
          process(vb, base + 64);
        }
      } else {
        uint32_t va[32], vb[32];
        int row_next = cnt > 0 ? tile_row(0) : 0;
        for (int tb = 0; tb < cnt; ++tb) {
          const int base = row_next + half * 64;
          if (tb + 1 < cnt) row_next = tile_row(tb + 1);
          wait_epi(&acc_full[as], aph);
          tc_fence_after();
          const uint32_t col = (uint32_t)((as * 2 + h) * kRows + half * 64);
          tmem_ld32(lane_addr + col, va);
          tmem_ld32(lane_addr + col + 32, vb);
          tmem_ld_wait();
          tc_fence_before();
          __syncwarp();
          if (lane == 0) mbar_arrive(&acc_empty[as]);
          if (++as == kAccStages) { as = 0; aph ^= 1u; }
          process(va, base);
          process(vb, base + 32);
        }
      }
      if constexpr (kSplit >= 2) {
        const int pair_bar = 1 + lg + 4 * h;
        asm volatile("bar.sync %0, 64;" ::"r"(pair_bar) : "memory");
        if (half == 0) {
          float cd[kC]; int ci[kC];
#pragma unroll
          for (int c = 0; c < kC; ++c) { cd[c] = l_cd[c * kEpiThreads]; ci[c] = l_ci[c * kEpiThreads]; }
#pragma unroll
          for (int b = 0; b < kC; ++b) {
            float d = l_cd[b * kEpiThreads + 128]; int i = l_ci[b * kEpiThreads + 128];
#pragma unroll
            for (int c = 0; c < kC; ++c) {
              if (d < cd[c]) { const float td = cd[c]; const int ti = ci[c]; cd[c] = d; ci[c] = i; d = td; i = ti; }
            }
          }
#pragma unroll
          for (int c = 0; c < kC; ++c) { l_cd[c * kEpiThreads] = cd[c]; l_ci[c * kEpiThreads] = ci[c]; }
        }
      }
      if (half == 0 && q_idx >= 0) {
#pragma unroll
        for (int c = 0; c < kKnnCand; ++c) {
          const int i = c < kC ? l_ci[c * kEpiThreads] : -1;
          cand_idx[q_idx * kKnnCand + c] = (i < 0 || !w.tperm) ? i : (i < n ? w.tperm[i] : -1);
        }
        cand_worst[q_idx] = l_cd[(kC - 1) * kEpiThreads];
      }
      if constexpr (kSplit >= 2) {
        asm volatile("bar.sync %0, 64;" ::"r"(1 + lg + 4 * h) : "memory");
      }
    }
  }
  tc_fence_before();
  __syncthreads();
  if (warp == 1) {
    tc_fence_after();
    asm volatile("tcgen05.dealloc.cta_group::1.sync.aligned.b32 %0, %1;" ::"r"(tmem_base), "r"((uint32_t)kTmemCols) : "memory");
  }
}


constexpr int kPruneThreads = kUnitQ;
constexpr double kPruneRel = 1e-9;
constexpr double kPruneSlack = 1e-13;

__device__ __forceinline__ double prune_project(const double* __restrict__ x, const KnnPruneGeom* __restrict__ g, int d, int na,
                                                double* __restrict__ p) {
  double c[kPruneMaxDim];
  double l1 = 0.0;
#pragma unroll
  for (int j = 0; j < kPruneMaxDim; ++j) { c[j] = j < d ? x[j] - g->mean[j] : 0.0; l1 += fabs(c[j]); }
#pragma unroll
  for (int a = 0; a < kPruneMaxDim; ++a) {
    if (a >= na) break;
    double s = 0.0;
    for (int j = 0; j < d; ++j) s += c[j] * g->axis[a][j];
    p[a] = s;
  }
  return l1;
}

__global__ void knn_prune_keys_kernel(const double* __restrict__ q, int64_t m, const KnnPruneGeom* __restrict__ g,
                                      unsigned* __restrict__ keys, int* __restrict__ vals) {
  const int64_t i = (int64_t)blockIdx.x * blockDim.x + threadIdx.x;
  if (i >= m) return;
  const int d = g->d, na = d < 3 ? d : 3;
  double p[kPruneMaxDim];
  prune_project(q + i * d, g, d, na, p);
  unsigned code = 0;
  for (int a = 0; a < na; ++a) {
    const double t = (p[a] - g->key_lo[a]) * g->key_scale[a];
    const unsigned v = t >= 0.0 ? (t < 1023.0 ? (unsigned)t : 1023u) : 0u;
#pragma unroll
    for (int b = 0; b < 10; ++b) code |= ((v >> b) & 1u) << (3 * b + 2 - a);
  }
  keys[i] = code;
  vals[i] = (int)i;
}

__device__ __forceinline__ double block_max(double v, double* sh) {
  v = warp_reduce(v, [](double a, double b) { return fmax(a, b); });
  __syncthreads();
  if ((threadIdx.x & 31) == 0) sh[threadIdx.x >> 5] = v;
  __syncthreads();
  double r = sh[0];
  for (int w = 1; w < kPruneThreads / 32; ++w) r = fmax(r, sh[w]);
  return r;
}

__global__ void __launch_bounds__(kPruneThreads)
knn_prune_unit_box_kernel(const double* __restrict__ q, int64_t m, const KnnPruneGeom* __restrict__ g, const int* __restrict__ qperm,
                          const float* __restrict__ qnorm, float qnorm_limit, double* __restrict__ ulo, double* __restrict__ uhi,
                          double* __restrict__ uslack) {
  __shared__ double s_lo[kPruneThreads / 32][kPruneMaxDim], s_hi[kPruneThreads / 32][kPruneMaxDim], s_red[kPruneThreads / 32];
  const int u = blockIdx.x, d = g->d, w = threadIdx.x >> 5, lane = threadIdx.x & 31;
  const int64_t pos = (int64_t)u * kUnitQ + threadIdx.x;
  const int64_t qi = pos < m ? qperm[pos] : -1;
  const bool valid = qi >= 0 && qnorm[qi] <= qnorm_limit;
  double p[kPruneMaxDim], l1 = 0.0;
  if (valid) l1 = prune_project(q + qi * d, g, d, d, p);
#pragma unroll
  for (int a = 0; a < kPruneMaxDim; ++a) {
    if (a >= d) break;
    const double lo = warp_reduce(valid ? p[a] : INFINITY, [](double x, double y) { return fmin(x, y); });
    const double hi = warp_reduce(valid ? p[a] : -INFINITY, [](double x, double y) { return fmax(x, y); });
    if (lane == 0) { s_lo[w][a] = lo; s_hi[w][a] = hi; }
  }
  const double l1max = block_max(l1, s_red);
  if (threadIdx.x < d) {
    double lo = INFINITY, hi = -INFINITY;
    for (int ww = 0; ww < kPruneThreads / 32; ++ww) { lo = fmin(lo, s_lo[ww][threadIdx.x]); hi = fmax(hi, s_hi[ww][threadIdx.x]); }
    ulo[(int64_t)u * d + threadIdx.x] = lo;
    uhi[(int64_t)u * d + threadIdx.x] = hi;
  }
  if (threadIdx.x == 0) uslack[u] = kPruneSlack * (1.0 + l1max);
}

__device__ __forceinline__ bool less_dt(double da, int ta, double db, int tb) { return da < db || (da == db && ta < tb); }

__global__ void __launch_bounds__(kPruneThreads)
knn_prune_seed_kernel(int t_tiles, int d, const double* __restrict__ ulo, const double* __restrict__ uhi, const double* __restrict__ tlo,
                      const double* __restrict__ thi, int S, int* __restrict__ seed, int* __restrict__ seed_cnt) {
  __shared__ double s_d[kPruneThreads / 32];
  __shared__ int s_t[kPruneThreads / 32];
  __shared__ int s_win;
  const int u = blockIdx.x, w = threadIdx.x >> 5, lane = threadIdx.x & 31;
  double c[kPruneMaxDim];
  for (int a = 0; a < d; ++a) c[a] = 0.5 * (ulo[(int64_t)u * d + a] + uhi[(int64_t)u * d + a]);
  double bd[kPruneSeedTiles];
  int bt[kPruneSeedTiles];
#pragma unroll
  for (int s = 0; s < kPruneSeedTiles; ++s) { bd[s] = INFINITY; bt[s] = INT_MAX; }
  for (int t = threadIdx.x; t < t_tiles; t += kPruneThreads) {
    double dd = 0.0;
    for (int a = 0; a < d; ++a) { const double x = c[a] - 0.5 * (tlo[(int64_t)t * d + a] + thi[(int64_t)t * d + a]); dd += x * x; }
    if (!(dd < INFINITY)) dd = INFINITY;
    int s = kPruneSeedTiles - 1;
    if (!less_dt(dd, t, bd[s], bt[s])) continue;
    while (s > 0 && less_dt(dd, t, bd[s - 1], bt[s - 1])) { bd[s] = bd[s - 1]; bt[s] = bt[s - 1]; --s; }
    bd[s] = dd; bt[s] = t;
  }
  for (int r = 0; r < S; ++r) {
    double md = bd[0];
    int mt = bt[0];
#pragma unroll
    for (int o = 16; o > 0; o >>= 1) {
      const double od = __shfl_xor_sync(0xffffffffu, md, o);
      const int ot = __shfl_xor_sync(0xffffffffu, mt, o);
      if (less_dt(od, ot, md, mt)) { md = od; mt = ot; }
    }
    if (lane == 0) { s_d[w] = md; s_t[w] = mt; }
    __syncthreads();
    if (threadIdx.x == 0) {
      for (int ww = 1; ww < kPruneThreads / 32; ++ww) if (less_dt(s_d[ww], s_t[ww], md, mt)) { md = s_d[ww]; mt = s_t[ww]; }
      s_win = mt;
      seed[(int64_t)u * S + r] = mt;
    }
    __syncthreads();
    if (bt[0] == s_win) {
#pragma unroll
      for (int s = 0; s + 1 < kPruneSeedTiles; ++s) { bd[s] = bd[s + 1]; bt[s] = bt[s + 1]; }
      bd[kPruneSeedTiles - 1] = INFINITY; bt[kPruneSeedTiles - 1] = INT_MAX;
    }
  }
  if (threadIdx.x == 0) seed_cnt[u] = S;
}

__global__ void __launch_bounds__(kPruneThreads)
knn_prune_bound_kernel(const double* __restrict__ train, const double* __restrict__ q, int64_t m, int d, int k,
                       const int* __restrict__ qperm, const int* __restrict__ cand_idx, const float* __restrict__ qnorm, float qnorm_limit,
                       const double* __restrict__ caller_bound, double* __restrict__ bound, double* __restrict__ unit_rad) {
  __shared__ double s_red[kPruneThreads / 32];
  const int u = blockIdx.x;
  const int64_t pos = (int64_t)u * kUnitQ + threadIdx.x;
  const int64_t qi = pos < m ? qperm[pos] : -1;
  const bool valid = qi >= 0 && qnorm[qi] <= qnorm_limit;
  double U = INFINITY;
  if (qi >= 0) {
    double best[kKnnCand];
    int nb = 0;
    for (int c = 0; c < kKnnCand; ++c) {
      const int i = cand_idx[qi * kKnnCand + c];
      if (i < 0) continue;
      double dd = 0.0;
      for (int j = 0; j < d; ++j) { const double x = q[qi * d + j] - train[(int64_t)i * d + j]; dd += x * x; }
      int s = nb++;
      while (s > 0 && dd < best[s - 1]) { best[s] = best[s - 1]; --s; }
      best[s] = dd;
    }
    if (nb >= k) U = best[k - 1];
    if (caller_bound) U = fmin(U, caller_bound[qi]);
    bound[qi] = U;
  }
  const double any = block_max(valid ? 1.0 : 0.0, s_red);
  const double r = block_max(valid ? U : -INFINITY, s_red);
  if (threadIdx.x == 0) unit_rad[u] = any > 0.0 ? r : INFINITY;
}

__global__ void __launch_bounds__(kPruneThreads)
knn_prune_list_kernel(int t_tiles, int d, const double* __restrict__ ulo, const double* __restrict__ uhi, const double* __restrict__ uslack,
                      const double* __restrict__ unit_rad, const double* __restrict__ tlo, const double* __restrict__ thi,
                      const double* __restrict__ tslack, int* __restrict__ tiles, int* __restrict__ count, int* __restrict__ unit_ids,
                      unsigned long long* __restrict__ kept) {
  using Scan = cub::BlockScan<int, kPruneThreads>;
  __shared__ typename Scan::TempStorage scan_tmp;
  __shared__ double s_lo[kPruneMaxDim], s_hi[kPruneMaxDim];
  const int u = blockIdx.x;
  if (threadIdx.x < d) { s_lo[threadIdx.x] = ulo[(int64_t)u * d + threadIdx.x]; s_hi[threadIdx.x] = uhi[(int64_t)u * d + threadIdx.x]; }
  __syncthreads();
  const double lim = unit_rad[u] * (1.0 + kPruneRel), sl_u = uslack[u];
  int run = 0;
  for (int base = 0; base < t_tiles; base += kPruneThreads) {
    const int t = base + threadIdx.x;
    int keep = 0;
    if (t < t_tiles) {
      const double sl = sl_u + tslack[t];
      double lb = 0.0;
      for (int a = 0; a < d; ++a) {
        const double gap = fmax(tlo[(int64_t)t * d + a] - s_hi[a], s_lo[a] - thi[(int64_t)t * d + a]) - sl;
        if (gap > 0.0) lb += gap * gap;
      }
      keep = lb <= lim;
    }
    int at, total;
    Scan(scan_tmp).ExclusiveSum(keep, at, total);
    if (keep) tiles[(int64_t)u * t_tiles + run + at] = t;
    run += total;
    __syncthreads();
  }
  if (threadIdx.x == 0) {
    count[u] = run;
    unit_ids[u] = u;
    atomicAdd(kept, (unsigned long long)run);
  }
}

}

float knn_tc16_max_norm() { return 8192.f; }
int64_t knn_tc16_padded_rows(int64_t rows, bool query) { const int b = query ? kUnitQ : kRows; return (rows + b - 1) / b * b; }
size_t knn_tc16_packed_bytes(int64_t rows, bool query) { return (size_t)(knn_tc16_padded_rows(rows, query) / kRows) * kTileBytes; }

cudaError_t knn_tc16_pack(const double* x, int64_t rows, int d, bool query, void* packed, float* norms, int* flags, cudaStream_t st,
                          const int* gather) {
  cudaMemsetAsync(flags, 0, 2 * sizeof(int), st);
  const int64_t rp = knn_tc16_padded_rows(rows, query);
  if (rp == 0) return cudaSuccess;
  knn_tc16_pack_kernel<<<(unsigned)((rp + 127) / 128), 128, 0, st>>>(x, rows, rp, d, query, static_cast<unsigned char*>(packed), norms,
                                                                    flags, knn_tc16_max_norm(), gather);
  return cudaGetLastError();
}

cudaError_t knn_tc16_filter(const void* qpacked, const void* tpacked, int64_t m, int64_t n, int k, const int* qflags, int* cand_idx,
                            float* cand_worst, int sm_count, cudaStream_t st, const float* thr0, const Tc16Work& work) {
  if (m == 0) return cudaSuccess;
  const int units = (int)(knn_tc16_padded_rows(m, true) / kUnitQ), t_tiles = (int)(knn_tc16_padded_rows(n, false) / kRows);
  static const int debug = [] { const char* e = std::getenv("DSP_TC16_DEBUG"); return e ? std::atoi(e) & 3 : 0; }();
  static const int force_c = [] { const char* e = std::getenv("DSP_TC16_CAND"); return e ? std::atoi(e) : 0; }();
  const bool small = force_c ? force_c < kKnnCand : k <= 3;
  auto fn = debug == 1 ? knn_tc16_filter_kernel<1, 5> : debug == 2 ? knn_tc16_filter_kernel<2, 5> : debug == 3 ? knn_tc16_filter_kernel<3, 5>
            : (small ? knn_tc16_filter_kernel<0, 5> : knn_tc16_filter_kernel<0, kKnnCand>);
  cudaError_t e = cudaFuncSetAttribute(fn, cudaFuncAttributeMaxDynamicSharedMemorySize, (int)kTcSmem);
  if (e != cudaSuccess) return e;
  const int grid = units < sm_count ? units : sm_count;
  if (work.counter) cudaMemsetAsync(work.counter, 0, sizeof(int), st);
  fn<<<grid, kTcThreads, kTcSmem, st>>>(static_cast<const unsigned char*>(qpacked), static_cast<const unsigned char*>(tpacked), m, (int)n,
                                        units, t_tiles, qflags, cand_idx, cand_worst, thr0, work);
  return cudaGetLastError();
}

}

namespace dsp {

namespace {

void jacobi_eigen(int d, double a[kPruneMaxDim][kPruneMaxDim], double v[kPruneMaxDim][kPruneMaxDim]) {
  for (int i = 0; i < d; ++i)
    for (int j = 0; j < d; ++j) v[i][j] = i == j ? 1.0 : 0.0;
  for (int sweep = 0; sweep < 100; ++sweep) {
    double off = 0.0, diag = 0.0;
    for (int p = 0; p < d; ++p) {
      diag += a[p][p] * a[p][p];
      for (int q = p + 1; q < d; ++q) off += a[p][q] * a[p][q];
    }
    if (!(off > 1e-32 * diag)) break;
    for (int p = 0; p < d; ++p)
      for (int q = p + 1; q < d; ++q) {
        if (a[p][q] == 0.0) continue;
        const double theta = (a[q][q] - a[p][p]) / (2.0 * a[p][q]);
        const double t = std::fabs(theta) > 1e150 ? 0.5 / theta : (theta >= 0 ? 1.0 : -1.0) / (std::fabs(theta) + std::sqrt(theta * theta + 1.0));
        const double c = 1.0 / std::sqrt(t * t + 1.0), s = t * c;
        for (int k = 0; k < d; ++k) { const double x = a[k][p], y = a[k][q]; a[k][p] = c * x - s * y; a[k][q] = s * x + c * y; }
        for (int k = 0; k < d; ++k) { const double x = a[p][k], y = a[q][k]; a[p][k] = c * x - s * y; a[q][k] = s * x + c * y; }
        for (int k = 0; k < d; ++k) { const double x = v[k][p], y = v[k][q]; v[k][p] = c * x - s * y; v[k][q] = s * x + c * y; }
      }
  }
}

struct PruneScratch {
  unsigned* keys[2];
  int* vals[2];
  void* sort_tmp;
  size_t sort_bytes;
  double *ulo, *uhi, *uslack, *rad;
  int *seed, *seed_cnt, *tiles, *count[2], *ids[2], *counter;
  unsigned long long* kept;
};

size_t prune_layout(int64_t m, int64_t n, unsigned char* base, PruneScratch& s) {
  const int64_t units = knn_tc16_padded_rows(m, true) / kUnitQ, t_tiles = knn_tc16_padded_rows(n, false) / kRows;
  size_t b1 = 0, b2 = 0;
  cub::DeviceRadixSort::SortPairs(nullptr, b1, (const unsigned*)nullptr, (unsigned*)nullptr, (const int*)nullptr, (int*)nullptr, (int)m, 0, 30);
  cub::DeviceRadixSort::SortPairsDescending(nullptr, b2, (const int*)nullptr, (int*)nullptr, (const int*)nullptr, (int*)nullptr, (int)units);
  s.sort_bytes = std::max(b1, b2);
  size_t off = 0;
  auto take = [&](size_t bytes) { void* p = base ? base + off : nullptr; off += (bytes + 255) / 256 * 256; return p; };
  for (int i = 0; i < 2; ++i) { s.keys[i] = (unsigned*)take(4 * (size_t)m); s.vals[i] = (int*)take(4 * (size_t)m); }
  s.sort_tmp = take(s.sort_bytes);
  s.ulo = (double*)take(8 * (size_t)units * kPruneMaxDim);
  s.uhi = (double*)take(8 * (size_t)units * kPruneMaxDim);
  s.uslack = (double*)take(8 * (size_t)units);
  s.rad = (double*)take(8 * (size_t)units);
  s.seed = (int*)take(4 * (size_t)units * kPruneSeedTiles);
  s.seed_cnt = (int*)take(4 * (size_t)units);
  s.tiles = (int*)take(4 * (size_t)units * t_tiles);
  for (int i = 0; i < 2; ++i) { s.count[i] = (int*)take(4 * (size_t)units); s.ids[i] = (int*)take(4 * (size_t)units); }
  s.counter = (int*)take(4);
  s.kept = (unsigned long long*)take(8);
  return off;
}

}

void knn_prune_plan(const double* x, int64_t n, int d, KnnPrunePlan& plan) {
  KnnPruneGeom& g = plan.geom;
  std::memset(&g, 0, sizeof g);
  g.d = d;
  for (int j = 0; j < d; ++j) {
    double s = 0.0;
    for (int64_t i = 0; i < n; ++i) s += x[i * d + j];
    g.mean[j] = s / (double)n;
  }
  double cov[kPruneMaxDim][kPruneMaxDim] = {}, vec[kPruneMaxDim][kPruneMaxDim];
  for (int64_t i = 0; i < n; ++i)
    for (int p = 0; p < d; ++p)
      for (int q = p; q < d; ++q) cov[p][q] += (x[i * d + p] - g.mean[p]) * (x[i * d + q] - g.mean[q]);
  for (int p = 0; p < d; ++p)
    for (int q = p; q < d; ++q) cov[q][p] = cov[p][q] /= (double)n;
  jacobi_eigen(d, cov, vec);
  int order[kPruneMaxDim];
  std::iota(order, order + d, 0);
  std::stable_sort(order, order + d, [&](int a, int b) { return cov[a][a] > cov[b][b]; });
  for (int a = 0; a < d; ++a)
    for (int j = 0; j < d; ++j) g.axis[a][j] = vec[j][order[a]];
  std::vector<double> pr((size_t)n * d), l1((size_t)n);
  for (int64_t i = 0; i < n; ++i) {
    double c[kPruneMaxDim], s1 = 0.0;
    for (int j = 0; j < d; ++j) { c[j] = x[i * d + j] - g.mean[j]; s1 += std::fabs(c[j]); }
    l1[(size_t)i] = s1;
    for (int a = 0; a < d; ++a) {
      double s = 0.0;
      for (int j = 0; j < d; ++j) s += c[j] * g.axis[a][j];
      pr[(size_t)i * d + a] = s;
    }
  }
  const int64_t t_tiles = knn_tc16_padded_rows(n, false) / kRows;
  plan.perm.resize((size_t)n);
  std::iota(plan.perm.begin(), plan.perm.end(), 0);
  int* perm = plan.perm.data();
  std::vector<std::pair<int64_t, int64_t>> stack{{0, t_tiles}};
  while (!stack.empty()) {
    const auto [t0, t1] = stack.back();
    stack.pop_back();
    if (t1 - t0 < 2) continue;
    const int64_t r0 = t0 * kRows, r1 = std::min<int64_t>(t1 * kRows, n), tm = t0 + (t1 - t0) / 2, rm = tm * kRows;
    int axis = 0;
    double widest = -1.0;
    for (int a = 0; a < d; ++a) {
      double lo = INFINITY, hi = -INFINITY;
      for (int64_t r = r0; r < r1; ++r) { const double v = pr[(size_t)perm[r] * d + a]; lo = std::min(lo, v); hi = std::max(hi, v); }
      if (hi - lo > widest) { widest = hi - lo; axis = a; }
    }
    std::nth_element(perm + r0, perm + rm, perm + r1, [&](int i, int j) {
      const double a = pr[(size_t)i * d + axis], b = pr[(size_t)j * d + axis];
      return a < b || (a == b && i < j);
    });
    stack.push_back({t0, tm});
    stack.push_back({tm, t1});
  }
  plan.lo.assign((size_t)t_tiles * d, INFINITY);
  plan.hi.assign((size_t)t_tiles * d, -INFINITY);
  plan.slack.assign((size_t)t_tiles, 0.0);
  for (int64_t r = 0; r < n; ++r) {
    const int64_t t = r / kRows, i = perm[r];
    for (int a = 0; a < d; ++a) {
      plan.lo[(size_t)t * d + a] = std::min(plan.lo[(size_t)t * d + a], pr[(size_t)i * d + a]);
      plan.hi[(size_t)t * d + a] = std::max(plan.hi[(size_t)t * d + a], pr[(size_t)i * d + a]);
    }
    plan.slack[(size_t)t] = std::max(plan.slack[(size_t)t], kPruneSlack * (1.0 + l1[(size_t)i]));
  }
  for (int a = 0; a < 3 && a < d; ++a) {
    double lo = INFINITY, hi = -INFINITY;
    for (int64_t t = 0; t < t_tiles; ++t) { lo = std::min(lo, plan.lo[(size_t)t * d + a]); hi = std::max(hi, plan.hi[(size_t)t * d + a]); }
    g.key_lo[a] = lo;
    g.key_scale[a] = hi > lo ? 1024.0 / (hi - lo) : 0.0;
  }
}

size_t knn_prune_scratch_bytes(int64_t m, int64_t n) {
  PruneScratch s;
  return prune_layout(m, n, nullptr, s);
}

cudaError_t knn_prune_prepare(const double* q, int64_t m, int64_t n, int d, int k, const double* train, const KnnPruneGeom* geom,
                              const int* tperm, const double* tile_lo, const double* tile_hi, const double* tile_slack, const void* tpacked,
                              void* qpacked, float* qnorm, int* qflags, const double* caller_bound, double* bound, int* cand_idx,
                              float* cand_worst, void* scratch, bool auto_fallback, int sm_count, cudaStream_t st, Tc16Work& work) {
  if (m == 0) return cudaSuccess;
  PruneScratch s;
  prune_layout(m, n, static_cast<unsigned char*>(scratch), s);
  const int units = (int)(knn_tc16_padded_rows(m, true) / kUnitQ), t_tiles = (int)(knn_tc16_padded_rows(n, false) / kRows);
  const float limit = knn_tc16_max_norm();
  knn_prune_keys_kernel<<<(unsigned)((m + 255) / 256), 256, 0, st>>>(q, m, geom, s.keys[0], s.vals[0]);
  size_t bytes = s.sort_bytes;
  cudaError_t e = cub::DeviceRadixSort::SortPairs(s.sort_tmp, bytes, s.keys[0], s.keys[1], s.vals[0], s.vals[1], (int)m, 0, 30, st);
  if (e != cudaSuccess) return e;
  const int* qperm = s.vals[1];
  if ((e = knn_tc16_pack(q, m, d, true, qpacked, qnorm, qflags, st, qperm)) != cudaSuccess) return e;
  knn_prune_unit_box_kernel<<<units, kPruneThreads, 0, st>>>(q, m, geom, qperm, qnorm, limit, s.ulo, s.uhi, s.uslack);
  const int S = std::min(kPruneSeedTiles, t_tiles);
  knn_prune_seed_kernel<<<units, kPruneThreads, 0, st>>>(t_tiles, d, s.ulo, s.uhi, tile_lo, tile_hi, S, s.seed, s.seed_cnt);
  Tc16Work seed;
  seed.tiles = s.seed; seed.tile_count = s.seed_cnt; seed.stride = S;
  seed.qperm = qperm; seed.tperm = tperm;
  if ((e = knn_tc16_filter(qpacked, tpacked, m, n, k, qflags, cand_idx, cand_worst, sm_count, st, nullptr, seed)) != cudaSuccess) return e;
  knn_prune_bound_kernel<<<units, kPruneThreads, 0, st>>>(train, q, m, d, k, qperm, cand_idx, qnorm, limit, caller_bound, bound, s.rad);
  cudaMemsetAsync(s.kept, 0, sizeof(unsigned long long), st);
  knn_prune_list_kernel<<<units, kPruneThreads, 0, st>>>(t_tiles, d, s.ulo, s.uhi, s.uslack, s.rad, tile_lo, tile_hi, tile_slack, s.tiles,
                                                         s.count[0], s.ids[0], s.kept);
  bytes = s.sort_bytes;
  e = cub::DeviceRadixSort::SortPairsDescending(s.sort_tmp, bytes, s.count[0], s.count[1], s.ids[0], s.ids[1], units, 0, 32, st);
  if (e != cudaSuccess) return e;
  work = Tc16Work();
  work.tiles = s.tiles; work.tile_count = s.count[0]; work.stride = t_tiles;
  work.unit_order = s.ids[1]; work.counter = s.counter;
  work.kept = s.kept;
  work.kept_limit = auto_fallback ? (unsigned long long)(0.85 * (double)units * (double)t_tiles) : ~0ull;
  work.qperm = qperm; work.tperm = tperm;
  return cudaGetLastError();
}

}
```

Baseline: 20.15 million.

## Split heavy KNN prune units into tile slices and merge partial top-k

Adds a schedule kernel that splits query units with long tile lists into slices spread across CTAs. Each slice writes partial candidate lists, and a new merge kernel combines them. This targets load imbalance where one CTA walks far more tiles than the others. It also replaces the brute-force seed-tile kernel with a kd-tree leaf lookup built on the host, and raises the seed tile count. The cost is an extra merge launch, extra scratch memory and more seed work.

```diff
diff --git a/dsp_audioreclabs_b200/csrc/capi.cu b/dsp_audioreclabs_b200/csrc/capi.cu
--- a/dsp_audioreclabs_b200/csrc/capi.cu
+++ b/dsp_audioreclabs_b200/csrc/capi.cu
@@ -1,3 +1,4 @@
+#include <algorithm>
 #include <cmath>
 #include <cstdarg>
 #include <cstdio>
@@ -851,7 +852,7 @@
     const size_t box = sizeof(double) * plan.lo.size();
     if (h->tc_train.ensure(knn_tc16_packed_bytes(n, false)) != cudaSuccess || h->tc_flags.ensure(64) != cudaSuccess ||
         h->prune_perm.ensure(sizeof(int) * (size_t)n) != cudaSuccess || h->prune_geom.ensure(sizeof(KnnPruneGeom)) != cudaSuccess ||
-        h->prune_box.ensure(2 * box + sizeof(double) * plan.slack.size()) != cudaSuccess)
+        h->prune_box.ensure(2 * box + sizeof(double) * plan.slack.size() + sizeof(KnnPruneNode) * plan.nodes.size()) != cudaSuccess)
       return bail(fail(DSP_ERR_NOMEM, "device allocation failed"));
     unsigned char* pb = h->prune_box.as<unsigned char>();
     cudaMemcpyAsync(h->prune_perm.p, plan.perm.data(), sizeof(int) * (size_t)n, cudaMemcpyHostToDevice, c->stream);
@@ -859,6 +860,9 @@
     cudaMemcpyAsync(pb, plan.lo.data(), box, cudaMemcpyHostToDevice, c->stream);
     cudaMemcpyAsync(pb + box, plan.hi.data(), box, cudaMemcpyHostToDevice, c->stream);
     cudaMemcpyAsync(pb + 2 * box, plan.slack.data(), sizeof(double) * plan.slack.size(), cudaMemcpyHostToDevice, c->stream);
+    if (!plan.nodes.empty())
+      cudaMemcpyAsync(pb + 2 * box + sizeof(double) * plan.slack.size(), plan.nodes.data(), sizeof(KnnPruneNode) * plan.nodes.size(),
+                      cudaMemcpyHostToDevice, c->stream);
     if (h->tc_train_rows.ensure(knn_tc16_packed_bytes(n, false)) != cudaSuccess) return bail(fail(DSP_ERR_NOMEM, "device allocation failed"));
     cudaError_t e = knn_tc16_pack(h->train64.as<double>(), n, d, false, h->tc_train_rows.p, nullptr, h->tc_flags.as<int>(), c->stream);
     if (e == cudaSuccess)
@@ -927,8 +931,10 @@
   dsp_context* c = h->ctx;
   CU(cudaSetDevice(c->device));
   CU(h->redo_list.ensure(sizeof(int32_t) * (size_t)m));
-  const unsigned long long* prune_kept = nullptr;
+  const unsigned long long *prune_kept = nullptr, *prune_seed_visits = nullptr;
+  const int* prune_cta_visits = nullptr;
   int64_t prune_visits = 0;
+  int prune_grid = 0;
   if (h->dp) {
     CU(h->cand_idx.ensure(sizeof(int) * (size_t)m * kKnnCand));
     CU(h->cand_worst.ensure(sizeof(float) * (size_t)m));
@@ -947,19 +953,23 @@
       const void* tpacked = h->tc_train_rows.p;
       const bool prune = c->knn_prune && knn_tc16_padded_rows(m, true) / kTc16UnitQueries * h->prune_tiles <= INT32_MAX;
       if (prune) {
-        CU(h->prune_ws.ensure(knn_prune_scratch_bytes(m, h->n)));
+        CU(h->prune_ws.ensure(knn_prune_scratch_bytes(m, h->n, c->sm_count)));
         CU(h->prune_bound.ensure(sizeof(double) * (size_t)m));
         CU(h->thr0.ensure(sizeof(float) * (size_t)m));
         const unsigned char* pb = h->prune_box.as<unsigned char>();
         const size_t box = sizeof(double) * (size_t)h->prune_tiles * h->d;
-        CU(knn_prune_prepare(q, m, h->n, h->d, h->k, h->train64.as<double>(), h->prune_geom.as<KnnPruneGeom>(), h->prune_perm.as<int>(),
-                             (const double*)pb, (const double*)(pb + box), (const double*)(pb + 2 * box), h->tc_train.p, h->tc_q.p,
-                             h->qnorm.as<float>(), qflags, bound, h->prune_bound.as<double>(), h->cand_idx.as<int>(),
-                             h->cand_worst.as<float>(), h->prune_ws.p, c->knn_prune == 1, c->sm_count, c->stream, work));
+        const KnnPruneNode* nodes = (const KnnPruneNode*)(pb + 2 * box + sizeof(double) * (size_t)h->prune_tiles);
+        CU(knn_prune_prepare(q, m, h->n, h->d, h->k, h->train64.as<double>(), h->prune_geom.as<KnnPruneGeom>(), nodes,
+                             h->prune_perm.as<int>(), (const double*)pb, (const double*)(pb + box), (const double*)(pb + 2 * box),
+                             h->tc_train.p, h->tc_q.p, h->qnorm.as<float>(), qflags, bound, h->prune_bound.as<double>(),
+                             h->cand_idx.as<int>(), h->cand_worst.as<float>(), h->prune_ws.p, c->knn_prune == 1, c->sm_count,
+                             c->stream, work, &prune_seed_visits));
         tpacked = h->tc_train.p;
         rerank_bound = h->prune_bound.as<double>();
         prune_kept = work.kept;
+        prune_cta_visits = work.cta_visits;
         prune_visits = knn_tc16_padded_rows(m, true) / kTc16UnitQueries * h->prune_tiles;
+        prune_grid = (int)std::min<int64_t>(knn_tc16_padded_rows(m, true) / kTc16UnitQueries, c->sm_count);
         CU(knn_bound_thresholds(rerank_bound, h->qnorm.as<float>(), m, err_rel, err_floor, h->thr0.as<float>(), c->stream));
         thr0 = h->thr0.as<float>();
         c->launches += 12;
@@ -975,7 +985,7 @@
       }
       CU(knn_tc16_filter(h->tc_q.p, tpacked, m, h->n, h->k, qflags, h->cand_idx.as<int>(), h->cand_worst.as<float>(),
                          c->sm_count, c->stream, thr0, work));
-      c->launches += 2;
+      c->launches += work.items ? 3 : 2;
     } else {
       CU(knn_scan(h->dp, h->train32.as<float>(), h->n, q, m, h->d, h->cand_idx.as<int>(), h->cand_worst.as<float>(),
                   h->qnorm.as<float>(), nullptr, c->stream));
@@ -1047,10 +1057,15 @@
     cudaStreamSynchronize(c->stream);
     fprintf(stderr, "[knn] m=%lld n=%lld exhaustive=%d refined=%d refined->exhaustive=%d\n", (long long)m, (long long)h->n, cnt[0], cnt[1], cnt[2]);
     if (prune_kept) {
-      unsigned long long kept = 0;
+      unsigned long long kept = 0, seed_visits = 0;
+      std::vector<int> cta((size_t)prune_grid);
       cudaMemcpyAsync(&kept, prune_kept, sizeof kept, cudaMemcpyDeviceToHost, c->stream);
+      cudaMemcpyAsync(&seed_visits, prune_seed_visits, sizeof seed_visits, cudaMemcpyDeviceToHost, c->stream);
+      cudaMemcpyAsync(cta.data(), prune_cta_visits, sizeof(int) * cta.size(), cudaMemcpyDeviceToHost, c->stream);
       cudaStreamSynchronize(c->stream);
-      fprintf(stderr, "[knn] prune: tile visits kept=%llu of %lld (%s)\n", kept, (long long)prune_visits,
+      const int busiest = cta.empty() ? 0 : *std::max_element(cta.begin(), cta.end());
+      fprintf(stderr, "[knn] prune: tile visits kept=%llu of %lld, seed visits=%llu, busiest CTA=%d (%s)\n", kept, (long long)prune_visits,
+              seed_visits, busiest,
               c->knn_prune == 1 && kept > (unsigned long long)(0.85 * (double)prune_visits) ? "every tile walked" : "lists walked");
     }
   }
diff --git a/dsp_audioreclabs_b200/csrc/knn.cuh b/dsp_audioreclabs_b200/csrc/knn.cuh
--- a/dsp_audioreclabs_b200/csrc/knn.cuh
+++ b/dsp_audioreclabs_b200/csrc/knn.cuh
@@ -55,29 +55,46 @@
   unsigned long long kept_limit = 0;
   const int* qperm = nullptr;
   const int* tperm = nullptr;
+  const int4* items = nullptr;
+  const int* item_count = nullptr;
+  const int* unit_slices = nullptr;
+  const int* unit_slot = nullptr;
+  float* part_cd = nullptr;
+  int* part_ci = nullptr;
+  int* cta_visits = nullptr;
 };
+int knn_tc16_cand(int k);
 cudaError_t knn_tc16_filter(const void* qpacked, const void* tpacked, int64_t m, int64_t n, int k, const int* qflags, int* cand_idx,
                             float* cand_worst, int sm_count, cudaStream_t st, const float* thr0 = nullptr, const Tc16Work& work = Tc16Work());
 
 constexpr int kPruneMaxDim = 15;
-constexpr int kPruneSeedTiles = 4;
+constexpr int kPruneSeedTiles = 16;
 struct KnnPruneGeom {
   int d;
+  int root;
   double mean[kPruneMaxDim];
   double axis[kPruneMaxDim][kPruneMaxDim];
   double key_lo[3], key_scale[3];
+};
+struct KnnPruneNode {
+  double split;
+  int axis;
+  int child[2];
 };
 struct KnnPrunePlan {
   KnnPruneGeom geom;
   std::vector<int> perm;
   std::vector<double> lo, hi, slack;
+  std::vector<KnnPruneNode> nodes;
 };
 void knn_prune_plan(const double* train, int64_t n, int d, KnnPrunePlan& plan);
-size_t knn_prune_scratch_bytes(int64_t m, int64_t n);
+size_t knn_prune_scratch_bytes(int64_t m, int64_t n, int sm_count);
 cudaError_t knn_prune_prepare(const double* q, int64_t m, int64_t n, int d, int k, const double* train, const KnnPruneGeom* geom,
-                              const int* tperm, const double* tile_lo, const double* tile_hi, const double* tile_slack, const void* tpacked,
-                              void* qpacked, float* qnorm, int* qflags, const double* caller_bound, double* bound, int* cand_idx,
-                              float* cand_worst, void* scratch, bool auto_fallback, int sm_count, cudaStream_t st, Tc16Work& work);
+                              const KnnPruneNode* nodes, const int* tperm, const double* tile_lo, const double* tile_hi,
+                              const double* tile_slack, const void* tpacked, void* qpacked, float* qnorm, int* qflags,
+                              const double* caller_bound, double* bound, int* cand_idx, float* cand_worst, void* scratch,
+                              bool auto_fallback, int sm_count, cudaStream_t st, Tc16Work& work,
+                              const unsigned long long** seed_visits = nullptr);
 cudaError_t knn_bound_thresholds(const double* bound, const float* qnorm, int64_t m, double err_rel, double err_floor, float* thr0,
                                  cudaStream_t st);
 
diff --git a/dsp_audioreclabs_b200/csrc/knn_tc16.cu b/dsp_audioreclabs_b200/csrc/knn_tc16.cu
--- a/dsp_audioreclabs_b200/csrc/knn_tc16.cu
+++ b/dsp_audioreclabs_b200/csrc/knn_tc16.cu
@@ -259,13 +259,30 @@
       int s = 0; uint32_t ph = 0;
       int qb = 0; uint32_t qph = 0;
       const bool lists = w.tiles && !(w.kept && *w.kept > w.kept_limit);
+      const bool sliced = lists && w.items;
+      const int n_work = sliced ? *w.item_count : units;
+      int visits = 0;
       for (int i = 0;; ++i) {
         wait(&q_empty[qb], qph ^ 1u);
         const int slot = w.counter ? atomicAdd(w.counter, 1) : (int)blockIdx.x + i * (int)gridDim.x;
-        const int u = slot < units ? (w.unit_order ? w.unit_order[slot] : slot) : -1;
-        const int cnt = (u >= 0 && lists) ? w.tile_count[u] : t_tiles, list = (u >= 0 && lists) ? u * w.stride : -1;
-        s_info[qb] = make_int4(u, cnt, list, 0);
-        if (u < 0) { mbar_arrive(&q_full[qb]); break; }
+        int4 item = make_int4(-1, 0, -1, -1);
+        if (slot < n_work) {
+          if (sliced) {
+            const int4 it = w.items[slot];
+            item = make_int4(it.x, it.z, it.x * w.stride + it.y, it.w);
+          } else {
+            const int u = w.unit_order ? w.unit_order[slot] : slot;
+            item = make_int4(u, lists ? w.tile_count[u] : t_tiles, lists ? u * w.stride : -1, -1);
+          }
+        }
+        const int u = item.x, cnt = item.y, list = item.z;
+        s_info[qb] = item;
+        if (u < 0) {
+          mbar_arrive(&q_full[qb]);
+          if (w.cta_visits) w.cta_visits[blockIdx.x] = visits;
+          break;
+        }
+        visits += cnt;
         mbar_expect_tx(&q_full[qb], (uint32_t)kQBufBytes);
         bulk_g2s(smem_u32(s_q + (size_t)qb * kQBufBytes), qpacked + (size_t)u * kQBufBytes, kQBufBytes, &q_full[qb]);
         if (++qb == 2) { qb = 0; qph ^= 1u; }
@@ -350,7 +367,7 @@
       __syncwarp();
       if (lane == 0) mbar_arrive(&q_empty[qb]);
       if (++qb == 2) { qb = 0; qph ^= 1u; }
-      const int u = info.x, cnt = info.y, list = info.z;
+      const int u = info.x, cnt = info.y, list = info.z, part = info.w;
       if (u < 0) break;
       auto tile_row = [&](int j) { return (list < 0 ? j : w.tiles[list + j]) * kRows; };
 #pragma unroll
@@ -470,12 +487,22 @@
         }
       }
       if (half == 0 && q_idx >= 0) {
-#pragma unroll
-        for (int c = 0; c < kKnnCand; ++c) {
-          const int i = c < kC ? l_ci[c * kEpiThreads] : -1;
-          cand_idx[q_idx * kKnnCand + c] = (i < 0 || !w.tperm) ? i : (i < n ? w.tperm[i] : -1);
-        }
-        cand_worst[q_idx] = l_cd[(kC - 1) * kEpiThreads];
+        if (part < 0) {
+#pragma unroll
+          for (int c = 0; c < kKnnCand; ++c) {
+            const int i = c < kC ? l_ci[c * kEpiThreads] : -1;
+            cand_idx[q_idx * kKnnCand + c] = (i < 0 || !w.tperm) ? i : (i < n ? w.tperm[i] : -1);
+          }
+          cand_worst[q_idx] = l_cd[(kC - 1) * kEpiThreads];
+        } else {
+          const int pos = (int)(q_own - (int64_t)u * kUnitQ);
+#pragma unroll
+          for (int c = 0; c < kC; ++c) {
+            const int i = l_ci[c * kEpiThreads];
+            w.part_ci[((size_t)part * kKnnCand + c) * kUnitQ + pos] = (i < 0 || !w.tperm) ? i : (i < n ? w.tperm[i] : -1);
+            w.part_cd[((size_t)part * kKnnCand + c) * kUnitQ + pos] = l_cd[c * kEpiThreads];
+          }
+        }
       }
       if constexpr (kSplit >= 2) {
         asm volatile("bar.sync %0, 64;" ::"r"(1 + lg + 4 * h) : "memory");
@@ -488,6 +515,35 @@
     tc_fence_after();
     asm volatile("tcgen05.dealloc.cta_group::1.sync.aligned.b32 %0, %1;" ::"r"(tmem_base), "r"((uint32_t)kTmemCols) : "memory");
   }
+}
+
+template <int kC>
+__global__ void __launch_bounds__(kUnitQ)
+knn_tc16_merge_kernel(int64_t m, const Tc16Work w, int* __restrict__ cand_idx, float* __restrict__ cand_worst) {
+  if (w.kept && *w.kept > w.kept_limit) return;
+  const int u = blockIdx.x, ns = w.unit_slices[u];
+  const int64_t pos = (int64_t)u * kUnitQ + threadIdx.x;
+  if (ns < 2 || pos >= m) return;
+  const int64_t qi = w.qperm ? (int64_t)w.qperm[pos] : pos;
+  float cd[kC]; int ci[kC];
+#pragma unroll
+  for (int c = 0; c < kC; ++c) { cd[c] = INFINITY; ci[c] = -1; }
+  for (int s = 0; s < ns; ++s) {
+    const size_t base = (size_t)(w.unit_slot[u] + s) * kKnnCand * kUnitQ + threadIdx.x;
+#pragma unroll
+    for (int b = 0; b < kC; ++b) {
+      float d = w.part_cd[base + (size_t)b * kUnitQ];
+      if (!(d < cd[kC - 1])) break;
+      int i = w.part_ci[base + (size_t)b * kUnitQ];
+#pragma unroll
+      for (int c = 0; c < kC; ++c) {
+        if (d < cd[c]) { const float td = cd[c]; const int ti = ci[c]; cd[c] = d; ci[c] = i; d = td; i = ti; }
+      }
+    }
+  }
+#pragma unroll
+  for (int c = 0; c < kKnnCand; ++c) cand_idx[qi * kKnnCand + c] = c < kC ? ci[c] : -1;
+  cand_worst[qi] = cd[kC - 1];
 }
 
 
@@ -540,16 +596,25 @@
 }
 
 __global__ void __launch_bounds__(kPruneThreads)
-knn_prune_unit_box_kernel(const double* __restrict__ q, int64_t m, const KnnPruneGeom* __restrict__ g, const int* __restrict__ qperm,
-                          const float* __restrict__ qnorm, float qnorm_limit, double* __restrict__ ulo, double* __restrict__ uhi,
-                          double* __restrict__ uslack) {
+knn_prune_unit_box_kernel(const double* __restrict__ q, int64_t m, const KnnPruneGeom* __restrict__ g, const KnnPruneNode* __restrict__ nodes,
+                          const int* __restrict__ qperm, const float* __restrict__ qnorm, float qnorm_limit, double* __restrict__ ulo,
+                          double* __restrict__ uhi, double* __restrict__ uslack, int* __restrict__ seed, int* __restrict__ seed_cnt,
+                          unsigned long long* __restrict__ seed_visits) {
   __shared__ double s_lo[kPruneThreads / 32][kPruneMaxDim], s_hi[kPruneThreads / 32][kPruneMaxDim], s_red[kPruneThreads / 32];
+  __shared__ int s_leaf[kPruneThreads], s_cnt[kPruneThreads];
   const int u = blockIdx.x, d = g->d, w = threadIdx.x >> 5, lane = threadIdx.x & 31;
   const int64_t pos = (int64_t)u * kUnitQ + threadIdx.x;
   const int64_t qi = pos < m ? qperm[pos] : -1;
   const bool valid = qi >= 0 && qnorm[qi] <= qnorm_limit;
   double p[kPruneMaxDim], l1 = 0.0;
-  if (valid) l1 = prune_project(q + qi * d, g, d, d, p);
+  int leaf = -1;
+  if (valid) {
+    l1 = prune_project(q + qi * d, g, d, d, p);
+    int node = g->root;
+    while (node >= 0) { const KnnPruneNode& nd = nodes[node]; node = nd.child[p[nd.axis] < nd.split ? 0 : 1]; }
+    leaf = ~node;
+  }
+  s_leaf[threadIdx.x] = leaf;
 #pragma unroll
   for (int a = 0; a < kPruneMaxDim; ++a) {
     if (a >= d) break;
@@ -564,57 +629,30 @@
     ulo[(int64_t)u * d + threadIdx.x] = lo;
     uhi[(int64_t)u * d + threadIdx.x] = hi;
   }
-  if (threadIdx.x == 0) uslack[u] = kPruneSlack * (1.0 + l1max);
-}
-
-__device__ __forceinline__ bool less_dt(double da, int ta, double db, int tb) { return da < db || (da == db && ta < tb); }
-
-__global__ void __launch_bounds__(kPruneThreads)
-knn_prune_seed_kernel(int t_tiles, int d, const double* __restrict__ ulo, const double* __restrict__ uhi, const double* __restrict__ tlo,
-                      const double* __restrict__ thi, int S, int* __restrict__ seed, int* __restrict__ seed_cnt) {
-  __shared__ double s_d[kPruneThreads / 32];
-  __shared__ int s_t[kPruneThreads / 32];
-  __shared__ int s_win;
-  const int u = blockIdx.x, w = threadIdx.x >> 5, lane = threadIdx.x & 31;
-  double c[kPruneMaxDim];
-  for (int a = 0; a < d; ++a) c[a] = 0.5 * (ulo[(int64_t)u * d + a] + uhi[(int64_t)u * d + a]);
-  double bd[kPruneSeedTiles];
-  int bt[kPruneSeedTiles];
-#pragma unroll
-  for (int s = 0; s < kPruneSeedTiles; ++s) { bd[s] = INFINITY; bt[s] = INT_MAX; }
-  for (int t = threadIdx.x; t < t_tiles; t += kPruneThreads) {
-    double dd = 0.0;
-    for (int a = 0; a < d; ++a) { const double x = c[a] - 0.5 * (tlo[(int64_t)t * d + a] + thi[(int64_t)t * d + a]); dd += x * x; }
-    if (!(dd < INFINITY)) dd = INFINITY;
-    int s = kPruneSeedTiles - 1;
-    if (!less_dt(dd, t, bd[s], bt[s])) continue;
-    while (s > 0 && less_dt(dd, t, bd[s - 1], bt[s - 1])) { bd[s] = bd[s - 1]; bt[s] = bt[s - 1]; --s; }
-    bd[s] = dd; bt[s] = t;
-  }
-  for (int r = 0; r < S; ++r) {
-    double md = bd[0];
-    int mt = bt[0];
-#pragma unroll
-    for (int o = 16; o > 0; o >>= 1) {
-      const double od = __shfl_xor_sync(0xffffffffu, md, o);
-      const int ot = __shfl_xor_sync(0xffffffffu, mt, o);
-      if (less_dt(od, ot, md, mt)) { md = od; mt = ot; }
-    }
-    if (lane == 0) { s_d[w] = md; s_t[w] = mt; }
-    __syncthreads();
-    if (threadIdx.x == 0) {
-      for (int ww = 1; ww < kPruneThreads / 32; ++ww) if (less_dt(s_d[ww], s_t[ww], md, mt)) { md = s_d[ww]; mt = s_t[ww]; }
-      s_win = mt;
-      seed[(int64_t)u * S + r] = mt;
-    }
-    __syncthreads();
-    if (bt[0] == s_win) {
-#pragma unroll
-      for (int s = 0; s + 1 < kPruneSeedTiles; ++s) { bd[s] = bd[s + 1]; bt[s] = bt[s + 1]; }
-      bd[kPruneSeedTiles - 1] = INFINITY; bt[kPruneSeedTiles - 1] = INT_MAX;
-    }
-  }
-  if (threadIdx.x == 0) seed_cnt[u] = S;
+  int votes = 0;
+  bool first = leaf >= 0;
+  if (leaf >= 0)
+    for (int j = 0; j < kPruneThreads; ++j) {
+      const int o = s_leaf[j];
+      votes += o == leaf;
+      if (o == leaf && j < (int)threadIdx.x) first = false;
+    }
+  s_cnt[threadIdx.x] = first ? votes : 0;
+  const int distinct = __syncthreads_count(first);
+  if (first) {
+    int rank = 0;
+    for (int j = 0; j < kPruneThreads; ++j) {
+      const int c = s_cnt[j];
+      rank += c > votes || (c == votes && s_leaf[j] < leaf);
+    }
+    if (rank < kPruneSeedTiles) seed[(int64_t)u * kPruneSeedTiles + rank] = leaf;
+  }
+  if (threadIdx.x == 0) {
+    const int ns = distinct < kPruneSeedTiles ? distinct : kPruneSeedTiles;
+    uslack[u] = kPruneSlack * (1.0 + l1max);
+    seed_cnt[u] = ns;
+    atomicAdd(seed_visits, (unsigned long long)ns);
+  }
 }
 
 __global__ void __launch_bounds__(kPruneThreads)
@@ -649,14 +687,20 @@
 }
 
 __global__ void __launch_bounds__(kPruneThreads)
-knn_prune_list_kernel(int t_tiles, int d, const double* __restrict__ ulo, const double* __restrict__ uhi, const double* __restrict__ uslack,
+knn_prune_list_kernel(const double* __restrict__ q, int64_t m, const KnnPruneGeom* __restrict__ g, const int* __restrict__ qperm,
+                      const float* __restrict__ qnorm, float qnorm_limit, const double* __restrict__ bound, int t_tiles,
+                      const double* __restrict__ ulo, const double* __restrict__ uhi, const double* __restrict__ uslack,
                       const double* __restrict__ unit_rad, const double* __restrict__ tlo, const double* __restrict__ thi,
                       const double* __restrict__ tslack, int* __restrict__ tiles, int* __restrict__ count, int* __restrict__ unit_ids,
                       unsigned long long* __restrict__ kept) {
   using Scan = cub::BlockScan<int, kPruneThreads>;
   __shared__ typename Scan::TempStorage scan_tmp;
   __shared__ double s_lo[kPruneMaxDim], s_hi[kPruneMaxDim];
-  const int u = blockIdx.x;
+  __shared__ int s_list[kPruneThreads], s_keep[kPruneThreads];
+  __shared__ double s_qp[kPruneMaxDim][kPruneThreads], s_qlim[kPruneThreads], s_qsl[kPruneThreads];
+  __shared__ double s_box[kPruneThreads / 32][32];
+  const int u = blockIdx.x, d = g->d, lane = threadIdx.x & 31;
+  int* list = tiles + (int64_t)u * t_tiles;
   if (threadIdx.x < d) { s_lo[threadIdx.x] = ulo[(int64_t)u * d + threadIdx.x]; s_hi[threadIdx.x] = uhi[(int64_t)u * d + threadIdx.x]; }
   __syncthreads();
   const double lim = unit_rad[u] * (1.0 + kPruneRel), sl_u = uslack[u];
@@ -675,15 +719,112 @@
     }
     int at, total;
     Scan(scan_tmp).ExclusiveSum(keep, at, total);
-    if (keep) tiles[(int64_t)u * t_tiles + run + at] = t;
+    if (keep) list[run + at] = t;
     run += total;
     __syncthreads();
+  }
+  constexpr int kQPL = kPruneThreads / 32;
+  const int64_t pos = (int64_t)u * kUnitQ + threadIdx.x;
+  const int64_t qi = pos < m ? qperm[pos] : -1;
+  const bool valid = qi >= 0 && qnorm[qi] <= qnorm_limit;
+  if (__syncthreads_or(valid)) {
+    {
+      double p[kPruneMaxDim] = {}, sl_q = 0.0, lim_q = -1.0;
+      if (valid) {
+        sl_q = kPruneSlack * (1.0 + prune_project(q + qi * d, g, d, d, p));
+        const double U = bound[qi];
+        lim_q = isnan(U) ? INFINITY : U * (1.0 + kPruneRel);
+      }
+#pragma unroll
+      for (int a = 0; a < kPruneMaxDim; ++a) s_qp[a][threadIdx.x] = p[a];
+      s_qlim[threadIdx.x] = lim_q;
+      s_qsl[threadIdx.x] = sl_q;
+    }
+    __syncthreads();
+    const int warp = threadIdx.x >> 5;
+    double lim_l[kQPL], sl_l[kQPL];
+#pragma unroll
+    for (int b = 0; b < kQPL; ++b) { lim_l[b] = s_qlim[lane + 32 * b]; sl_l[b] = s_qsl[lane + 32 * b]; }
+    double* box = s_box[warp];
+    int out = 0;
+    for (int base = 0; base < run; base += kPruneThreads) {
+      const int nb = min(kPruneThreads, run - base);
+      if ((int)threadIdx.x < nb) s_list[threadIdx.x] = list[base + threadIdx.x];
+      s_keep[threadIdx.x] = 0;
+      __syncthreads();
+      for (int j = warp; j < nb; j += kPruneThreads / 32) {
+        const int t = s_list[j];
+        if (lane <= 2 * d) box[lane] = lane < d ? tlo[(int64_t)t * d + lane] : lane < 2 * d ? thi[(int64_t)t * d + lane - d] : tslack[t];
+        __syncwarp();
+        const double sl_t = box[2 * d];
+        double lb[kQPL];
+#pragma unroll
+        for (int b = 0; b < kQPL; ++b) lb[b] = 0.0;
+        for (int a = 0; a < d; ++a) {
+          const double lo = box[a], hi = box[d + a];
+          bool live = false;
+#pragma unroll
+          for (int b = 0; b < kQPL; ++b) {
+            const double x = s_qp[a][lane + 32 * b];
+            const double gap = fmax(lo - x, x - hi) - (sl_l[b] + sl_t);
+            if (gap > 0.0) lb[b] += gap * gap;
+            live |= lb[b] <= lim_l[b];
+          }
+          if (!__any_sync(0xffffffffu, live)) break;
+        }
+        bool hit = false;
+#pragma unroll
+        for (int b = 0; b < kQPL; ++b) hit |= lb[b] <= lim_l[b];
+        if (__any_sync(0xffffffffu, hit) && lane == 0) s_keep[j] = 1;
+        __syncwarp();
+      }
+      __syncthreads();
+      const int keep = (int)threadIdx.x < nb && s_keep[threadIdx.x];
+      int at, total;
+      Scan(scan_tmp).ExclusiveSum(keep, at, total);
+      if (keep) list[out + at] = s_list[threadIdx.x];
+      out += total;
+      __syncthreads();
+    }
+    run = out;
   }
   if (threadIdx.x == 0) {
     count[u] = run;
     unit_ids[u] = u;
     atomicAdd(kept, (unsigned long long)run);
   }
+}
+
+constexpr int kPruneSliceMin = 64;
+constexpr int kScheduleThreads = 1024;
+__global__ void __launch_bounds__(kScheduleThreads)
+knn_prune_schedule_kernel(int units, int grid, const int* __restrict__ count, const int* __restrict__ order,
+                          const unsigned long long* __restrict__ kept, int4* __restrict__ items, int* __restrict__ item_count,
+                          int* __restrict__ unit_slices, int* __restrict__ unit_slot) {
+  using Scan = cub::BlockScan<int, kScheduleThreads>;
+  __shared__ typename Scan::TempStorage scan_tmp;
+  const unsigned long long per = (*kept + 4ull * grid - 1) / (4ull * grid);
+  const int S = per > (unsigned long long)kPruneSliceMin ? (int)per : kPruneSliceMin;
+  int item0 = 0, slot0 = 0;
+  for (int base = 0; base < units; base += kScheduleThreads) {
+    const int i = base + threadIdx.x;
+    int u = -1, c = 0, ns = 0;
+    if (i < units) { u = order[i]; c = count[u]; ns = c > S ? (c + S - 1) / S : 1; }
+    const int multi = ns > 1 ? ns : 0;
+    int io, so, itot, stot;
+    Scan(scan_tmp).ExclusiveSum(ns, io, itot);
+    __syncthreads();
+    Scan(scan_tmp).ExclusiveSum(multi, so, stot);
+    __syncthreads();
+    if (u >= 0) {
+      unit_slices[u] = ns;
+      unit_slot[u] = multi ? slot0 + so : -1;
+      for (int j = 0; j < ns; ++j) items[item0 + io + j] = make_int4(u, j * S, min(S, c - j * S), multi ? slot0 + so + j : -1);
+    }
+    item0 += itot;
+    slot0 += stot;
+  }
+  if (threadIdx.x == 0) *item_count = item0;
 }
 
 }
@@ -707,8 +848,7 @@
   if (m == 0) return cudaSuccess;
   const int units = (int)(knn_tc16_padded_rows(m, true) / kUnitQ), t_tiles = (int)(knn_tc16_padded_rows(n, false) / kRows);
   static const int debug = [] { const char* e = std::getenv("DSP_TC16_DEBUG"); return e ? std::atoi(e) & 3 : 0; }();
-  static const int force_c = [] { const char* e = std::getenv("DSP_TC16_CAND"); return e ? std::atoi(e) : 0; }();
-  const bool small = force_c ? force_c < kKnnCand : k <= 3;
+  const bool small = knn_tc16_cand(k) < kKnnCand;
   auto fn = debug == 1 ? knn_tc16_filter_kernel<1, 5> : debug == 2 ? knn_tc16_filter_kernel<2, 5> : debug == 3 ? knn_tc16_filter_kernel<3, 5>
             : (small ? knn_tc16_filter_kernel<0, 5> : knn_tc16_filter_kernel<0, kKnnCand>);
   cudaError_t e = cudaFuncSetAttribute(fn, cudaFuncAttributeMaxDynamicSharedMemorySize, (int)kTcSmem);
@@ -717,7 +857,16 @@
   if (work.counter) cudaMemsetAsync(work.counter, 0, sizeof(int), st);
   fn<<<grid, kTcThreads, kTcSmem, st>>>(static_cast<const unsigned char*>(qpacked), static_cast<const unsigned char*>(tpacked), m, (int)n,
                                         units, t_tiles, qflags, cand_idx, cand_worst, thr0, work);
+  if (work.items) {
+    if (debug || small) knn_tc16_merge_kernel<5><<<units, kUnitQ, 0, st>>>(m, work, cand_idx, cand_worst);
+    else knn_tc16_merge_kernel<kKnnCand><<<units, kUnitQ, 0, st>>>(m, work, cand_idx, cand_worst);
+  }
   return cudaGetLastError();
+}
+
+int knn_tc16_cand(int k) {
+  static const int force_c = [] { const char* e = std::getenv("DSP_TC16_CAND"); return e ? std::atoi(e) : 0; }();
+  return (force_c ? force_c < kKnnCand : k <= 3) ? 5 : kKnnCand;
 }
 
 }
@@ -756,10 +905,13 @@
   size_t sort_bytes;
   double *ulo, *uhi, *uslack, *rad;
   int *seed, *seed_cnt, *tiles, *count[2], *ids[2], *counter;
-  unsigned long long* kept;
+  unsigned long long *kept, *seed_visits;
+  int4* items;
+  int *item_count, *unit_slices, *unit_slot, *part_ci, *cta_visits;
+  float* part_cd;
 };
 
-size_t prune_layout(int64_t m, int64_t n, unsigned char* base, PruneScratch& s) {
+size_t prune_layout(int64_t m, int64_t n, int sm_count, unsigned char* base, PruneScratch& s) {
   const int64_t units = knn_tc16_padded_rows(m, true) / kUnitQ, t_tiles = knn_tc16_padded_rows(n, false) / kRows;
   size_t b1 = 0, b2 = 0;
   cub::DeviceRadixSort::SortPairs(nullptr, b1, (const unsigned*)nullptr, (unsigned*)nullptr, (const int*)nullptr, (int*)nullptr, (int)m, 0, 30);
@@ -779,6 +931,15 @@
   for (int i = 0; i < 2; ++i) { s.count[i] = (int*)take(4 * (size_t)units); s.ids[i] = (int*)take(4 * (size_t)units); }
   s.counter = (int*)take(4);
   s.kept = (unsigned long long*)take(8);
+  s.seed_visits = (unsigned long long*)take(8);
+  const size_t slots = 8 * (size_t)sm_count;
+  s.items = (int4*)take(16 * ((size_t)units + 4 * (size_t)sm_count));
+  s.item_count = (int*)take(4);
+  s.unit_slices = (int*)take(4 * (size_t)units);
+  s.unit_slot = (int*)take(4 * (size_t)units);
+  s.part_cd = (float*)take(4 * slots * kKnnCand * kUnitQ);
+  s.part_ci = (int*)take(4 * slots * kKnnCand * kUnitQ);
+  s.cta_visits = (int*)take(4 * (size_t)sm_count);
   return off;
 }
 
@@ -820,11 +981,16 @@
   plan.perm.resize((size_t)n);
   std::iota(plan.perm.begin(), plan.perm.end(), 0);
   int* perm = plan.perm.data();
-  std::vector<std::pair<int64_t, int64_t>> stack{{0, t_tiles}};
+  plan.nodes.clear();
+  struct Range { int64_t t0, t1; int parent, side; };
+  std::vector<Range> stack{{0, t_tiles, -1, 0}};
   while (!stack.empty()) {
-    const auto [t0, t1] = stack.back();
+    const Range rg = stack.back();
+    const int64_t t0 = rg.t0, t1 = rg.t1;
     stack.pop_back();
-    if (t1 - t0 < 2) continue;
+    const int id = t1 - t0 < 2 ? ~(int)t0 : (int)plan.nodes.size();
+    (rg.parent < 0 ? g.root : plan.nodes[(size_t)rg.parent].child[rg.side]) = id;
+    if (id < 0) continue;
     const int64_t r0 = t0 * kRows, r1 = std::min<int64_t>(t1 * kRows, n), tm = t0 + (t1 - t0) / 2, rm = tm * kRows;
     int axis = 0;
     double widest = -1.0;
@@ -837,8 +1003,9 @@
       const double a = pr[(size_t)i * d + axis], b = pr[(size_t)j * d + axis];
       return a < b || (a == b && i < j);
     });
-    stack.push_back({t0, tm});
-    stack.push_back({tm, t1});
+    plan.nodes.push_back({pr[(size_t)perm[rm] * d + axis], axis, {0, 0}});
+    stack.push_back({t0, tm, id, 0});
+    stack.push_back({tm, t1, id, 1});
   }
   plan.lo.assign((size_t)t_tiles * d, INFINITY);
   plan.hi.assign((size_t)t_tiles * d, -INFINITY);
@@ -859,19 +1026,21 @@
   }
 }
 
-size_t knn_prune_scratch_bytes(int64_t m, int64_t n) {
+size_t knn_prune_scratch_bytes(int64_t m, int64_t n, int sm_count) {
   PruneScratch s;
-  return prune_layout(m, n, nullptr, s);
+  return prune_layout(m, n, sm_count, nullptr, s);
 }
 
 cudaError_t knn_prune_prepare(const double* q, int64_t m, int64_t n, int d, int k, const double* train, const KnnPruneGeom* geom,
-                              const int* tperm, const double* tile_lo, const double* tile_hi, const double* tile_slack, const void* tpacked,
-                              void* qpacked, float* qnorm, int* qflags, const double* caller_bound, double* bound, int* cand_idx,
-                              float* cand_worst, void* scratch, bool auto_fallback, int sm_count, cudaStream_t st, Tc16Work& work) {
+                              const KnnPruneNode* nodes, const int* tperm, const double* tile_lo, const double* tile_hi,
+                              const double* tile_slack, const void* tpacked, void* qpacked, float* qnorm, int* qflags,
+                              const double* caller_bound, double* bound, int* cand_idx, float* cand_worst, void* scratch,
+                              bool auto_fallback, int sm_count, cudaStream_t st, Tc16Work& work, const unsigned long long** seed_visits) {
   if (m == 0) return cudaSuccess;
   PruneScratch s;
-  prune_layout(m, n, static_cast<unsigned char*>(scratch), s);
+  prune_layout(m, n, sm_count, static_cast<unsigned char*>(scratch), s);
   const int units = (int)(knn_tc16_padded_rows(m, true) / kUnitQ), t_tiles = (int)(knn_tc16_padded_rows(n, false) / kRows);
+  const int grid = std::min(units, sm_count);
   const float limit = knn_tc16_max_norm();
   knn_prune_keys_kernel<<<(unsigned)((m + 255) / 256), 256, 0, st>>>(q, m, geom, s.keys[0], s.vals[0]);
   size_t bytes = s.sort_bytes;
@@ -879,26 +1048,33 @@
   if (e != cudaSuccess) return e;
   const int* qperm = s.vals[1];
   if ((e = knn_tc16_pack(q, m, d, true, qpacked, qnorm, qflags, st, qperm)) != cudaSuccess) return e;
-  knn_prune_unit_box_kernel<<<units, kPruneThreads, 0, st>>>(q, m, geom, qperm, qnorm, limit, s.ulo, s.uhi, s.uslack);
-  const int S = std::min(kPruneSeedTiles, t_tiles);
-  knn_prune_seed_kernel<<<units, kPruneThreads, 0, st>>>(t_tiles, d, s.ulo, s.uhi, tile_lo, tile_hi, S, s.seed, s.seed_cnt);
+  cudaMemsetAsync(s.seed_visits, 0, sizeof(unsigned long long), st);
+  knn_prune_unit_box_kernel<<<units, kPruneThreads, 0, st>>>(q, m, geom, nodes, qperm, qnorm, limit, s.ulo, s.uhi, s.uslack, s.seed,
+                                                             s.seed_cnt, s.seed_visits);
   Tc16Work seed;
-  seed.tiles = s.seed; seed.tile_count = s.seed_cnt; seed.stride = S;
+  seed.tiles = s.seed; seed.tile_count = s.seed_cnt; seed.stride = kPruneSeedTiles;
   seed.qperm = qperm; seed.tperm = tperm;
   if ((e = knn_tc16_filter(qpacked, tpacked, m, n, k, qflags, cand_idx, cand_worst, sm_count, st, nullptr, seed)) != cudaSuccess) return e;
   knn_prune_bound_kernel<<<units, kPruneThreads, 0, st>>>(train, q, m, d, k, qperm, cand_idx, qnorm, limit, caller_bound, bound, s.rad);
   cudaMemsetAsync(s.kept, 0, sizeof(unsigned long long), st);
-  knn_prune_list_kernel<<<units, kPruneThreads, 0, st>>>(t_tiles, d, s.ulo, s.uhi, s.uslack, s.rad, tile_lo, tile_hi, tile_slack, s.tiles,
-                                                         s.count[0], s.ids[0], s.kept);
+  knn_prune_list_kernel<<<units, kPruneThreads, 0, st>>>(q, m, geom, qperm, qnorm, limit, bound, t_tiles, s.ulo, s.uhi, s.uslack, s.rad,
+                                                         tile_lo, tile_hi, tile_slack, s.tiles, s.count[0], s.ids[0], s.kept);
   bytes = s.sort_bytes;
   e = cub::DeviceRadixSort::SortPairsDescending(s.sort_tmp, bytes, s.count[0], s.count[1], s.ids[0], s.ids[1], units, 0, 32, st);
   if (e != cudaSuccess) return e;
+  knn_prune_schedule_kernel<<<1, kScheduleThreads, 0, st>>>(units, grid, s.count[0], s.ids[1], s.kept, s.items, s.item_count,
+                                                            s.unit_slices, s.unit_slot);
   work = Tc16Work();
   work.tiles = s.tiles; work.tile_count = s.count[0]; work.stride = t_tiles;
   work.unit_order = s.ids[1]; work.counter = s.counter;
   work.kept = s.kept;
   work.kept_limit = auto_fallback ? (unsigned long long)(0.85 * (double)units * (double)t_tiles) : ~0ull;
   work.qperm = qperm; work.tperm = tperm;
+  work.items = s.items; work.item_count = s.item_count;
+  work.unit_slices = s.unit_slices; work.unit_slot = s.unit_slot;
+  work.part_cd = s.part_cd; work.part_ci = s.part_ci;
+  work.cta_visits = s.cta_visits;
+  if (seed_visits) *seed_visits = s.seed_visits;
   return cudaGetLastError();
 }
 
```

New measurement: 20.02 million (median of 6 runs). No clear change (-0.7%).
